# akshathmangudi/KAN-ViT

Measured on AMD Instinct MI355X. Metric: images/sec (train step) KAN-ViT 224x224, higher is better.
Workload: dtype f32

## Files before the change

include/kanvit.h:

```cpp
#ifndef KANVIT_H
#define KANVIT_H

#include <stddef.h>
#include <stdint.h>

#ifdef __cplusplus
extern "C" {
#endif

#if defined(__GNUC__) || defined(__clang__)
#pragma GCC visibility push(default)
#endif

#define KANVIT_ABI_VERSION 7

#define KANVIT_OK 0
#define KANVIT_EINVAL (-22)
#define KANVIT_ENOMEM (-12)
#define KANVIT_EDEVICE (-5)

#define KANVIT_FLAG_BF16_MFMA 1

#define KANVIT_FLAG_UNIFORM_KNOTS 2
#define KANVIT_FLAG_FUSED_LN 8
#define KANVIT_FLAG_SHARED_BPARAMS 4

#define KANVIT_FLAG_SINE_DFREQ 16

#define KANVIT_LINEAR 0
#define KANVIT_CHEBY 1
#define KANVIT_BSPLINE 2
#define KANVIT_RBF 3
#define KANVIT_SINE 4
#define KANVIT_FOURIER 5

typedef struct kanvit_layer_desc {
    int32_t family;
    int32_t groups;
    int32_t x_group_mod;
    int32_t I;
    int32_t O;
    int32_t G;
    int32_t spline_order;
    int32_t has_base;
    float rbf_inv_h;
    int32_t flags;
    int64_t M;
    int64_t ldx;
    int64_t ldu;
    int64_t ldy;
    int64_t bparam_stride;
    float ln_eps;
    int32_t base_act;
} kanvit_layer_desc;


#define KANVIT_BASE_SILU 0
#define KANVIT_BASE_GELU 1
#define KANVIT_BASE_GELU_TANH 2
#define KANVIT_BASE_RELU 3
#define KANVIT_BASE_TANH 4
#define KANVIT_BASE_IDENTITY 5

int kanvit_layer_ln_fusable(const kanvit_layer_desc* d);

size_t kanvit_layer_ln_bwd_workspace(const kanvit_layer_desc* d);
int kanvit_layer_ln_bwd(const kanvit_layer_desc* d, const float* x, const float* stats, const float* bparams, const float* du,
                        float* dx, float* dgamma, float* dbeta, void* workspace, size_t workspace_bytes, void* stream);

size_t kanvit_layer_fwd_workspace(const kanvit_layer_desc* d);
int kanvit_layer_fwd(const kanvit_layer_desc* d, const float* x, const float* u, const float* w,
                     const float* bparams, const float* bias, float* y, void* workspace, size_t workspace_bytes,
                     void* stream);

size_t kanvit_layer_bwd_input_workspace(const kanvit_layer_desc* d);
int kanvit_layer_bwd_input(const kanvit_layer_desc* d, const float* x, const float* u, const float* w,
                           const float* bparams, const float* dy, float* dx, float* du, float* dparam,
                           void* workspace, size_t workspace_bytes, void* stream);
int64_t kanvit_layer_dparam_tiles(const kanvit_layer_desc* d);
int kanvit_layer_sine_dfreq_ok(const kanvit_layer_desc* d);

size_t kanvit_layer_bwd_weight_workspace(const kanvit_layer_desc* d);
int kanvit_layer_bwd_weight(const kanvit_layer_desc* d, const float* x, const float* u, const float* bparams,
                            const float* dy, float* dw, void* workspace, size_t workspace_bytes, void* stream);

int kanvit_edge_l1_supported(const kanvit_layer_desc* d);
int64_t kanvit_edge_l1_row_bands(const kanvit_layer_desc* d);
size_t kanvit_edge_l1_fwd_workspace(const kanvit_layer_desc* d);
int kanvit_edge_l1_fwd(const kanvit_layer_desc* d, const float* x, const float* w, const float* bparams, float* A, void* workspace,
                       size_t workspace_bytes, void* stream);
size_t kanvit_edge_l1_bwd_workspace(const kanvit_layer_desc* d);
int kanvit_edge_l1_bwd(const kanvit_layer_desc* d, const float* x, const float* w, const float* bparams, const float* gA, float* dw,
                       float* dx, void* workspace, size_t workspace_bytes, void* stream);

#define KANVIT_BSPLINE_REFIT_TAU 1e-5
int kanvit_bspline_refit_supported(const kanvit_layer_desc* d);
size_t kanvit_bspline_refit_workspace(const kanvit_layer_desc* d);
int kanvit_bspline_refit_gram(const kanvit_layer_desc* d, const float* x, const float* old_knots, const float* new_knots, double* N,
                              double* C, void* workspace, size_t workspace_bytes, void* stream);
int kanvit_bspline_refit_solve(const kanvit_layer_desc* d, const double* N, const double* C, const float* w_old, float* w_new,
                               unsigned char* ok, void* stream);

int kanvit_bspline_regrid_supported(const kanvit_layer_desc* d, int old_G);
size_t kanvit_bspline_regrid_workspace(const kanvit_layer_desc* d, int old_G);
int kanvit_bspline_regrid_gram(const kanvit_layer_desc* d, int old_G, const float* x, const float* old_knots, const float* new_knots,
                               double* N, double* C, void* workspace, size_t workspace_bytes, void* stream);
int kanvit_bspline_regrid_solve(const kanvit_layer_desc* d, int old_G, const double* N, const double* C, const float* w_old,
                                float* w_new, unsigned char* ok, void* stream);

typedef struct kanvit_patch_desc {
    int32_t C, H, W;
    int32_t n_patches;
    int32_t prepend_rows;
    int32_t reserved;
} kanvit_patch_desc;
int kanvit_patch_embed_fwd(const kanvit_layer_desc* d, const kanvit_patch_desc* p, const float* images, const float* w,
                           const float* bparams, const float* bias, const float* cls, const float* pos, float* y,
                           void* stream);
int kanvit_patch_embed_fwd_ws(const kanvit_layer_desc* d, const kanvit_patch_desc* p, const float* images, const float* w,
                              const float* bparams, const float* bias, const float* cls, const float* pos, float* y,
                              void* workspace, size_t workspace_bytes, void* stream);
int kanvit_patch_embed_bwd_weight_ok(const kanvit_layer_desc* d, const kanvit_patch_desc* p);
size_t kanvit_patch_embed_bwd_weight_workspace(const kanvit_layer_desc* d, const kanvit_patch_desc* p);
int kanvit_patch_embed_bwd_weight(const kanvit_layer_desc* d, const kanvit_patch_desc* p, const float* images,
                                  const float* bparams, const float* dy, float* dw, void* workspace, size_t workspace_bytes,
                                  void* stream);

#define KANVIT_ATTN_MAX_N 256
#define KANVIT_ATTN_MAX_D 64
typedef struct kanvit_attn_desc {
    int32_t B, H, N, D;
    int32_t causal;
    float scale;
    int32_t flags;
    int32_t reserved;
    int64_t q_stride_b, q_stride_h, q_stride_n;
    int64_t k_stride_b, k_stride_h, k_stride_n;
    int64_t v_stride_b, v_stride_h, v_stride_n;
    int64_t o_stride_b, o_stride_h, o_stride_n;
} kanvit_attn_desc;

int kanvit_attn_fwd(const kanvit_attn_desc* d, const float* q, const float* k, const float* v,
                    float* o, float* lse, void* stream);
size_t kanvit_attn_bwd_workspace(const kanvit_attn_desc* d);
int kanvit_attn_bwd(const kanvit_attn_desc* d, const float* q, const float* k, const float* v,
                    const float* o, const float* lse, const float* d_o,
                    float* dq, float* dk, float* dv, void* workspace, size_t workspace_bytes, void* stream);

#define KANVIT_ATTN_X_MAX_D 128
typedef struct kanvit_attn_ext {
    int32_t Nk;
    int32_t reserved;
    const void* mask;
    int64_t mask_stride_b, mask_stride_h, mask_stride_q, mask_stride_k;
} kanvit_attn_ext;
int kanvit_attn_x_fwd(const kanvit_attn_desc* d, const kanvit_attn_ext* e, const float* q, const float* k, const float* v,
                      float* o, float* lse, void* stream);
size_t kanvit_attn_x_bwd_workspace(const kanvit_attn_desc* d, const kanvit_attn_ext* e);
int kanvit_attn_x_bwd(const kanvit_attn_desc* d, const kanvit_attn_ext* e, const float* q, const float* k, const float* v,
                      const float* o, const float* lse, const float* d_o, float* dq, float* dk, float* dv, void* workspace,
                      size_t workspace_bytes, void* stream);

int kanvit_attn_probs(const kanvit_attn_desc* d, const kanvit_attn_ext* e, const float* q, const float* k, float* p,
                      int64_t p_stride_b, int64_t p_stride_h, int64_t p_stride_q, int32_t rows, void* stream);

int kanvit_attn_q1_fwd(const kanvit_attn_desc* d, const kanvit_attn_ext* e, const float* q, const float* k, const float* v,
                       float* o, float* p, void* stream);
int kanvit_attn_q1_bwd(const kanvit_attn_desc* d, const kanvit_attn_ext* e, const float* q, const float* k, const float* v,
                       const float* o, const float* p, const float* d_o, float* dq, float* dk, float* dv, void* stream);

int kanvit_ff_small_supported(int D, int F);
int64_t kanvit_ff_small_max_rows(void);
int kanvit_ff_small_fwd(int64_t M, int D, int F, const float* x, const float* w1, const float* b1, const float* w2, const float* b2,
                        float* y, void* stream);
size_t kanvit_ff_small_bwd_workspace(int64_t M, int D, int F);
int kanvit_ff_small_bwd(int64_t M, int D, int F, const float* x, const float* w1, const float* b1, const float* w2, const float* dy,
                        float* dx, float* dw1, float* db1, float* dw2, float* db2, void* workspace, size_t workspace_bytes, void* stream);
int kanvit_lnff_small_fwd(int64_t M, int D, int F, float eps, const float* x, const float* delta, const float* gamma, const float* beta,
                          const float* w1, const float* b1, const float* w2, const float* b2, float* s, float* mean, float* rstd, float* y,
                          void* stream);
int kanvit_lnff_small_bwd(int64_t M, int D, int F, const float* s, const float* mean, const float* rstd, const float* gamma, const float* beta,
                          const float* w1, const float* b1, const float* w2, const float* dy, const float* ds_in, float* ds, float* dgamma,
                          float* dbeta, float* dw1, float* db1, float* dw2, float* db2, void* workspace, size_t workspace_bytes, void* stream);

int kanvit_addln_fwd(int64_t M, int D, float eps, const float* x, const float* delta, const float* gamma, const float* beta,
                     float* xsum, float* y, float* mean, float* rstd, void* stream);
size_t kanvit_addln_bwd_workspace(int64_t M, int D);
int kanvit_addln_bwd(int64_t M, int D, const float* xsum, const float* gamma, const float* mean, const float* rstd,
                     const float* dy, const float* dres, float* dx, float* dgamma, float* dbeta, void* workspace,
                     size_t workspace_bytes, void* stream);
int kanvit_addln_fwd_ex(int64_t M, int D, float eps, const float* x, const void* delta, int delta_bf16, const float* gamma, const float* beta,
                        float* xsum, void* y, int y_bf16, float* mean, float* rstd, void* stream);
int kanvit_addln_bwd_ex(int64_t M, int D, const float* xsum, const float* gamma, const float* mean, const float* rstd,
                        const void* dy, int dy_bf16, const float* dres, float* dx, void* dx_bf16, float* dgamma, float* dbeta, void* workspace,
                        size_t workspace_bytes, void* stream);

#define KANVIT_DEPTH_MAX_BRANCHES 64
int kanvit_depth_scales(int64_t B, int n_branch, const float* keep, uint64_t seed, uint64_t* counter, float* scales, void* stream);
int kanvit_addln_sd_fwd(int64_t M, int D, float eps, const float* x, const void* delta, int delta_bf16, const float* gamma, const float* beta,
                        float* xsum, void* y, int y_bf16, float* mean, float* rstd, const float* row_scale, int64_t rows_per_sample,
                        void* stream);
int kanvit_addln_sd_bwd(int64_t M, int D, const float* xsum, const float* gamma, const float* mean, const float* rstd,
                        const void* dy, int dy_bf16, const float* dres, float* dx, void* ddelta, int ddelta_bf16, float* dgamma, float* dbeta,
                        const float* row_scale, int64_t rows_per_sample, void* workspace, size_t workspace_bytes, void* stream);

size_t kanvit_relu_bwd_bias_workspace(int64_t M, int N);
int kanvit_relu_bwd_bias(int64_t M, int N, const float* dy, const float* y, float* dh, float* dbias, void* workspace,
                         size_t workspace_bytes, void* stream);
int kanvit_relu_bwd_bias_bf16(int64_t M, int N, const void* dy_bf16, const void* y_bf16, void* dh_bf16, float* dbias, void* workspace,
                              size_t workspace_bytes, void* stream);

int kanvit_split3_bf16(int64_t M, int K, const float* x, const float* bias, int relu, const void* mask_hi, int64_t mask_ld,
                       void* out, int pattern, void* stream);

int kanvit_augment_u8_supported(int64_t N, int H, int W, int C, int pad_y, int pad_x);
int kanvit_augment_u8(const uint8_t* images, const int64_t* labels, const int64_t* idx, const float* lut, float* out, int64_t* y_out,
                      int32_t* params_out, int64_t N, int64_t B, int H, int W, int C, int pad_y, int pad_x, int flip, uint64_t seed,
                      uint64_t epoch, void* stream);

int kanvit_mix_u8(const uint8_t* images, const int64_t* labels, const int64_t* idx, const float* lut, const int64_t* partner,
                  const float* weight, const int32_t* box, float* out, int64_t* y_out, int64_t* y2_out, float* w_out, int64_t N, int64_t B,
                  int H, int W, int C, int pad_y, int pad_x, int flip, uint64_t seed, uint64_t epoch, void* stream);

int kanvit_resample_u8_supported(int64_t N, int H, int W, int C, int OH, int OW);
int kanvit_resample_u8(const uint8_t* images, const int64_t* labels, const int64_t* idx, const float* lut, const int32_t* crop,
                       const int64_t* partner, const float* weight, const int32_t* box, float* out, int64_t* y_out, int64_t* y2_out,
                       float* w_out, int64_t N, int64_t B, int H, int W, int C, int OH, int OW, void* stream);

int kanvit_soft_ce(const float* logits, int64_t ld, const int64_t* y1, const int64_t* y2, const float* w, int64_t B, int C, float eps,
                   float* loss_rows, float* dlogits, float* loss, void* stream);

int kanvit_metrics_update(const void* logits, int logits_bf16, int64_t ld, const int64_t* labels, int64_t B, int C, int64_t n0, int64_t cap,
                          float* probs_t, int32_t* labels_out, int32_t* preds_out, int64_t* confusion, void* stream);
size_t kanvit_metrics_auc_pairs_workspace(int64_t n, int C);
int kanvit_metrics_auc_pairs(const float* probs_t, const int32_t* labels, int64_t n, int C, int64_t cap, int64_t* counts, void* workspace,
                             size_t workspace_bytes, void* stream);

#define KANVIT_OPTIM_MAX_TENSORS 80
#define KANVIT_OPTIM_CHUNK 4096
int kanvit_optim_max_tensors(void);
size_t kanvit_optim_sumsq_workspace(int n, const int64_t* numel);
int kanvit_optim_sumsq(int n, const void* const* grads, const int64_t* numel, void* workspace, size_t workspace_bytes, void* stream);
int kanvit_optim_begin(const void* partials, int64_t n_partials, double max_norm, int64_t* step, float* norm_coef, void* stream);
int kanvit_optim_adamw(int n, void* const* params, const void* const* grads, const int64_t* offsets, const int64_t* numel,
                       const int32_t* decay, float* exp_avg, float* exp_avg_sq, float* ema, int64_t state_numel, const float* table,
                       int64_t table_rows, const int64_t* step, const float* norm_coef, int has_wd, float b1, float ob1, float b2, float ob2,
                       float eps, float d, float od, void* stream);

#define KANVIT_DECLARE_FAMILY(name)                                                                           \
    int kanvit_##name##_fwd(const kanvit_layer_desc*, const float*, const float*, const float*, const float*, \
                            const float*, float*, void*, size_t, void*);                                      \
    int kanvit_##name##_bwd_input(const kanvit_layer_desc*, const float*, const float*, const float*,         \
                                  const float*, const float*, float*, float*, float*, void*, size_t, void*);  \
    int kanvit_##name##_bwd_weight(const kanvit_layer_desc*, const float*, const float*, const float*,        \
                                   const float*, float*, void*, size_t, void*);                               \
    int kanvit_##name##_qkv_fwd(const kanvit_layer_desc*, const float*, const float*, const float*,           \
                                const float*, const float*, float*, void*, size_t, void*);                    \
    int kanvit_##name##_qkv_bwd_input(const kanvit_layer_desc*, const float*, const float*, const float*,     \
                                      const float*, const float*, float*, float*, float*, void*, size_t,      \
                                      void*);                                                                 \
    int kanvit_##name##_qkv_bwd_weight(const kanvit_layer_desc*, const float*, const float*, const float*,    \
                                       const float*, float*, void*, size_t, void*);
KANVIT_DECLARE_FAMILY(linear)
KANVIT_DECLARE_FAMILY(cheby)
KANVIT_DECLARE_FAMILY(bspline)
KANVIT_DECLARE_FAMILY(rbf)
KANVIT_DECLARE_FAMILY(sine)
KANVIT_DECLARE_FAMILY(fourier)

int kanvit_abi_version(void);
const char* kanvit_last_error(void);
const char* kanvit_config(void);
int kanvit_config_reload(void);
int kanvit_device_count(void);

#if defined(__GNUC__) || defined(__clang__)
#pragma GCC visibility pop
#endif

#ifdef __cplusplus
}
#endif
#endif
```

kan-vit_amd/csrc/attention.hip:

```cpp
#include "attention_common.h"

#include <type_traits>

#include <stdlib.h>

namespace {

constexpr int ATHR = 256;
constexpr float LOG2E = 1.4426950408889634f;

typedef __bf16 bf16x8_t __attribute__((ext_vector_type(8)));
typedef __bf16 bf16x2_t __attribute__((ext_vector_type(2)));
typedef unsigned u32x4 __attribute__((ext_vector_type(4)));

__device__ __forceinline__ unsigned kv_pk(float lo, float hi) {
    bf16x2_t v = {(__bf16)lo, (__bf16)hi};
    return __builtin_bit_cast(unsigned, v);
}
__device__ __forceinline__ bf16x8_t kv_pack8(const float (&f)[8]) {
    const u32x4 u = {kv_pk(f[0], f[1]), kv_pk(f[2], f[3]), kv_pk(f[4], f[5]), kv_pk(f[6], f[7])};
    return __builtin_bit_cast(bf16x8_t, u);
}
__device__ __forceinline__ bf16x8_t kv_row8(const float* __restrict__ p) {
    float f[8];
// ... 1973 lines not shown
    if (int rc = kv_launch<KV>(kv_name, p.grid, threads, p.lds, a, st)) return rc;
    return kv_launch<DQ>(dq_name, p.grid_q, threads, p.lds_q, a, st);
}

int launch_bwd(const AttnArgs& a, const AttnBwdPlan& p, hipStream_t st) {
    return kv_pick<1, 2>(a.D <= 32 ? 1 : 2, [&](auto dt) {
        constexpr int DT = decltype(dt)::value;
        switch (p.form) {
            case ATTN_BWD_KV4_DQ3:
                return kv_pick<4, 8>(p.nkt, [&](auto n) {
                    return launch_pair<attn_bwd_kv4_kernel<2>, attn_bwd_dq3_kernel<2, decltype(n)::value>>("attn_bwd_kv4_kernel", "attn_bwd_dq3_kernel", 512, a, p, st);
                });
            case ATTN_BWD_KV3_DQ3:
                return kv_pick<2, 4, 8>(p.nkt, [&](auto n) {
                    constexpr int NKT = decltype(n)::value;
                    return launch_pair<attn_bwd_kv3_kernel<DT, NKT>, attn_bwd_dq3_kernel<DT, NKT>>("attn_bwd_kv3_kernel", "attn_bwd_dq3_kernel", 512, a, p, st);
                });
            case ATTN_BWD_KV2DS_DQ:
                return launch_pair<attn_bwd_kv2_kernel<DT, false, true>, attn_bwd_dq_kernel<DT>>("attn_bwd_kv2_kernel", "attn_bwd_dq_kernel", 512, a, p, st);
            case ATTN_BWD_KV2DS_DQ_BF16:
                return kv_pick<4, 8>(p.nkt, [&](auto n) {
                    return launch_pair<attn_bwd_kv2_kernel<DT, true, true>, attn_bwd_dq_bf16_kernel<DT, decltype(n)::value>>("attn_bwd_kv2_kernel", "attn_bwd_dq_bf16_kernel", 512, a, p, st);
                });
            case ATTN_BWD_KV2_Q2:
                return p.bf16 ? launch_pair<attn_bwd_kv2_kernel<DT, true, false>, attn_bwd_q2_kernel<DT, true>>("attn_bwd_kv2_kernel", "attn_bwd_q2_kernel", 512, a, p, st)
                              : launch_pair<attn_bwd_kv2_kernel<DT, false, false>, attn_bwd_q2_kernel<DT, false>>("attn_bwd_kv2_kernel", "attn_bwd_q2_kernel", 512, a, p, st);
            default:
                return p.bf16 ? launch_pair<attn_bwd_kv_kernel<DT, true>, attn_bwd_q_kernel<DT, true>>("attn_bwd_kv_kernel", "attn_bwd_q_kernel", ATHR, a, p, st)
                              : launch_pair<attn_bwd_kv_kernel<DT, false>, attn_bwd_q_kernel<DT, false>>("attn_bwd_kv_kernel", "attn_bwd_q_kernel", ATHR, a, p, st);
        }
    });
}

__device__ __forceinline__ void attn_small_store_row(float* __restrict__ rowp, const f32x16& acc, int hf, int D, float mul) {
#pragma unroll
    for (int r = 0; r < 16; ++r) {
        const int d = kv_acc_row(r, hf);
        if (d < D) rowp[d] = acc[r] * mul;
    }
}

__global__ __launch_bounds__(256) void attn_small_fwd_kernel(const AttnArgs a) {
    const int lane = threadIdx.x & 63, wave = threadIdx.x >> 6, l31 = lane & 31, hf = lane >> 5;
    const int bh = blockIdx.x * 4 + wave;
    if (bh >= a.B * a.H) return;
    const int bi = bh / a.H, hi = bh - bi * a.H;
    const int N = a.N, D = a.D, DHc = (D + 1) / 2;
    const bool row_ok = l31 < N;
    const float* qrow = a.q + bi * a.qsb + hi * a.qsh + (long long)(row_ok ? l31 : 0) * a.qsn;
    const float* krow = a.k + bi * a.ksb + hi * a.ksh + (long long)(row_ok ? l31 : 0) * a.ksn;
    const float* vb = a.v + bi * a.vsb + hi * a.vsh;
    float vt[16];
#pragma unroll
    for (int r = 0; r < 16; ++r) {
        const int key = kv_acc_row(r, hf);
        vt[r] = (key < N && l31 < D) ? vb[(long long)key * a.vsn + l31] : 0.0f;
    }
    f32x16 sacc;
#pragma unroll
    for (int r = 0; r < 16; ++r) sacc[r] = 0.0f;
    for (int s = 0; s < DHc; ++s) {
        const int d = hf * DHc + s;
        const bool ok = row_ok && d < D;
        sacc = __builtin_amdgcn_mfma_f32_32x32x2f32(ok ? krow[d] : 0.0f, ok ? qrow[d] : 0.0f, sacc, 0, 0, 0);
    }
    const float sc2 = a.scale * LOG2E;
    float mx = -INFINITY;
#pragma unroll
    for (int r = 0; r < 16; ++r) {
        const int key = kv_acc_row(r, hf);
        if (key >= N || (a.causal && key > l31)) sacc[r] = -INFINITY;
        mx = fmaxf(mx, sacc[r]);
    }
    mx = fmaxf(mx, __shfl_xor(mx, 32));
    float sum = 0.0f;
#pragma unroll
    for (int r = 0; r < 16; ++r) {
        const float p = exp2f((sacc[r] - mx) * sc2);
        sacc[r] = p;
        sum += p;
    }
    sum += __shfl_xor(sum, 32);
    f32x16 oacc;
#pragma unroll
    for (int r = 0; r < 16; ++r) oacc[r] = 0.0f;
#pragma unroll
    for (int r = 0; r < 16; ++r) oacc = __builtin_amdgcn_mfma_f32_32x32x2f32(vt[r], sacc[r], oacc, 0, 0, 0);
    if (row_ok) {
        attn_small_store_row(a.out + bi * a.osb + hi * a.osh + (long long)l31 * a.osn, oacc, hf, D, 1.0f / sum);
        if (hf == 0 && a.lse) a.lse[(long long)bh * N + l31] = mx * a.scale + logf(sum);
    }
}

__global__ __launch_bounds__(256) void attn_small_bwd_kernel(const AttnArgs a) {
    __shared__ float tiles[4][2][32 * 33];
    const int lane = threadIdx.x & 63, wave = threadIdx.x >> 6, l31 = lane & 31, hf = lane >> 5;
    const int bh = blockIdx.x * 4 + wave;
    if (bh >= a.B * a.H) return;
    const int bi = bh / a.H, hi = bh - bi * a.H;
    const int N = a.N, D = a.D, DHc = (D + 1) / 2;
    const bool row_ok = l31 < N;
    const long long r0 = row_ok ? l31 : 0;
    const float* qb = a.q + bi * a.qsb + hi * a.qsh;
    const float* kb = a.k + bi * a.ksb + hi * a.ksh;
    const float* vb = a.v + bi * a.vsb + hi * a.vsh;
    const float* ob = a.o + bi * a.osb + hi * a.osh;
    const float* dob = a.d_o + bi * a.osb + hi * a.osh;
    float kt[16], dot[16], qt[16];
#pragma unroll
    for (int r = 0; r < 16; ++r) {
        const int key = kv_acc_row(r, hf);
        kt[r] = (key < N && l31 < D) ? kb[(long long)key * a.ksn + l31] : 0.0f;
        const int qq = 2 * r + hf;
        const bool ok = qq < N && l31 < D;
        dot[r] = ok ? dob[(long long)qq * a.osn + l31] : 0.0f;
        qt[r] = ok ? qb[(long long)qq * a.qsn + l31] : 0.0f;
    }
    f32x16 sacc, pacc;
#pragma unroll
    for (int r = 0; r < 16; ++r) {
        sacc[r] = 0.0f;
        pacc[r] = 0.0f;
    }
    float dl = 0.0f;
    for (int s = 0; s < DHc; ++s) {
        const int d = hf * DHc + s;
        const bool ok = row_ok && d < D;
        const float kv = ok ? kb[r0 * a.ksn + d] : 0.0f, qv = ok ? qb[r0 * a.qsn + d] : 0.0f;
        const float vv = ok ? vb[r0 * a.vsn + d] : 0.0f, dv = ok ? dob[r0 * a.osn + d] : 0.0f;
        const float ov = ok ? ob[r0 * a.osn + d] : 0.0f;
        sacc = __builtin_amdgcn_mfma_f32_32x32x2f32(kv, qv, sacc, 0, 0, 0);
        pacc = __builtin_amdgcn_mfma_f32_32x32x2f32(vv, dv, pacc, 0, 0, 0);
        dl += dv * ov;
    }
    dl += __shfl_xor(dl, 32);
    const float sc2 = a.scale * LOG2E;
    const float lse2 = row_ok ? a.lse_in[(long long)bh * N + l31] * LOG2E : INFINITY;
    float* pt = tiles[wave][0];
    float* dst = tiles[wave][1];
#pragma unroll
    for (int r = 0; r < 16; ++r) {
        const int key = kv_acc_row(r, hf);
        float p = exp2f(sacc[r] * sc2 - lse2);
        if (key >= N || (a.causal && key > l31)) p = 0.0f;
        const float ds = p * a.scale * (pacc[r] - dl);
        sacc[r] = p;
        pacc[r] = ds;
        pt[key * 33 + l31] = p;
        dst[key * 33 + l31] = ds;
    }
    f32x16 dqacc, dkacc, dvacc;
#pragma unroll
    for (int r = 0; r < 16; ++r) {
        dqacc[r] = 0.0f;
        dkacc[r] = 0.0f;
        dvacc[r] = 0.0f;
    }
#pragma unroll
    for (int r = 0; r < 16; ++r) dqacc = __builtin_amdgcn_mfma_f32_32x32x2f32(kt[r], pacc[r], dqacc, 0, 0, 0);
    __builtin_amdgcn_wave_barrier();
#pragma unroll
    for (int r = 0; r < 16; ++r) {
        dvacc = __builtin_amdgcn_mfma_f32_32x32x2f32(dot[r], pt[l31 * 33 + 2 * r + hf], dvacc, 0, 0, 0);
        dkacc = __builtin_amdgcn_mfma_f32_32x32x2f32(qt[r], dst[l31 * 33 + 2 * r + hf], dkacc, 0, 0, 0);
    }
    if (row_ok) {
        attn_small_store_row(a.dq + bi * a.qsb + hi * a.qsh + (long long)l31 * a.qsn, dqacc, hf, D, 1.0f);
        attn_small_store_row(a.dk + bi * a.ksb + hi * a.ksh + (long long)l31 * a.ksn, dkacc, hf, D, 1.0f);
        attn_small_store_row(a.dv + bi * a.vsb + hi * a.vsh + (long long)l31 * a.vsn, dvacc, hf, D, 1.0f);
    }
}

struct AttnSwitches {
    bool v1, v2, v3, v4, no_ds, no_bf16;
    int grid;
};
AttnSwitches attn_switches() {
    const KvConfig& c = kv_config();
    return {c.attn_v1 != 0, c.attn_v2 != 0, c.attn_v3 != 0, c.attn_v4 != 0, c.attn_no_ds != 0, c.no_bf16 != 0, c.attn_grid};
}

unsigned grid_per_cu(int nbh, int per_cu, int grid_override) {
    const int g = grid_override > 0 ? grid_override : KV_N_CU * per_cu;
    return (unsigned)(nbh < g ? nbh : g);
}
unsigned grid_resident(int nbh, size_t lds, int grid_override) { return grid_per_cu(nbh, lds * 2 <= 160 * 1024 ? 2 : 1, grid_override); }

int nkt_bucket(int nkt) { return nkt <= 2 ? nkt : nkt <= 4 ? 4 : nkt <= 7 ? 7 : 8; }

}

AttnFwdPlan plan_attn_fwd(const kanvit_attn_desc* d, uintptr_t align) {
    const AttnSwitches sw = attn_switches();
    const int nbh = d->B * d->H, nkt = (d->N + 31) / 32, D = d->D <= 32 ? 32 : 64;
    const size_t NP = (size_t)nkt * 32;
    AttnFwdPlan p{};
    if (d->N <= 32 && d->D <= 32 && !sw.v1 && !sw.v2) {
        p.form = ATTN_FWD_SMALL;
        p.grid = (unsigned)((nbh + 3) / 4);
        return p;
    }
    p.bf16 = (d->flags & KANVIT_FLAG_BF16_MFMA) && d->D % 16 == 0 && !sw.no_bf16;
    const bool rows16 = desc_vec(d) && align % 16 == 0;
    const bool newest = rows16 && !sw.v1 && !sw.v2 && !sw.v3;
    const int t16 = kv_attn16_tiles(d);
    if (newest && !sw.v4 && !d->causal && t16 && (!p.bf16 || t16 == KV_ATTN16_TILES)) {
        p.form = p.bf16 ? ATTN_FWD_16_BF16 : ATTN_FWD_16;
        p.nkt = t16;
        p.lds = kv_attn16_fwd_lds(d->N);
        p.grid = grid_per_cu(nbh, 1, sw.grid);
    } else if (newest && !p.bf16 && d->D == 64 && nkt >= 3 && nkt <= 7 && kv_a4_lds(d->N, 64) <= 160 * 1024) {
        p.form = ATTN_FWD_FOURTH;
        p.nkt = nkt <= 4 ? 4 : 7;
        p.lds = kv_a4_lds(d->N, 64);
        p.grid = grid_per_cu(nbh, 1, sw.grid);
    } else if (rows16 && !p.bf16 && d->D == D && !sw.v1 && !sw.v2 && nkt <= 7) {
        p.form = ATTN_FWD_THIRD;
        p.nkt = nkt_bucket(nkt);
        p.lds = sizeof(float) * 2 * NP * kv_pad4(D);
        p.grid = grid_resident(nbh, p.lds, sw.grid);
    } else if (rows16 && d->D == D && !sw.v1 && nkt <= 7) {
        p.form = ATTN_FWD_SECOND;
        p.nkt = nkt_bucket(nkt);
        p.lds = p.bf16 ? sizeof(unsigned short) * (NP * (D + 8) + D * (NP + 8)) : sizeof(float) * 2 * NP * (D + 1);
        p.grid = (unsigned)nbh;
    } else {
        p.form = ATTN_FWD_FIRST;
        p.nkt = nkt_bucket(nkt);
        p.lds = sizeof(float) * (2 * NP * (D + 1) + (size_t)4 * 32 * (D + 1));
        p.grid = (unsigned)nbh;
    }
    return p;
}

AttnBwdPlan plan_attn_bwd(const kanvit_attn_desc* d, const AttnAlign& al) {
    const AttnSwitches sw = attn_switches();
    const int nbh = d->B * d->H, nkt = (d->N + 31) / 32, D = d->D <= 32 ? 32 : 64;
    const size_t NP = (size_t)nkt * 32;
    AttnBwdPlan p{};
    p.bf16 = (d->flags & KANVIT_FLAG_BF16_MFMA) && d->D % 16 == 0 && !sw.no_bf16;
    const bool want16 = !sw.v1 && !sw.v2 && !sw.v3 && !sw.v4 && !sw.no_ds && d->D == 64 && !d->causal && (d->N + 15) / 16 == KV_ATTN16_TILES;
    const bool ds = (d->D == 32 || d->D == 64) && !d->causal && !sw.no_ds && !sw.v1 && !(want16 && !p.bf16) && (!p.bf16 || d->N <= 256);
    p.ws_bytes = (sizeof(float) * (size_t)d->B * d->H * d->N + 15) / 16 * 16 + (ds ? (p.bf16 ? sizeof(unsigned short) : sizeof(float)) * (size_t)d->B * d->H * NP * NP : 0);
    p.grid = p.grid_q = (unsigned)nbh;
    if (d->N <= 32 && d->D <= 32 && !sw.v1 && !sw.v2) {
        p.form = ATTN_BWD_SMALL;
        p.bf16 = false;
        p.grid = (unsigned)((nbh + 3) / 4);
        return p;
    }
    const bool rows16 = desc_vec(d) && al.rows % 16 == 0;
    if (want16 && rows16 && kv_attn16_tiles(d) && al.o % 16 == 0 && al.lse % 4 == 0) {
        p.form = p.bf16 ? ATTN_BWD_16_BF16 : ATTN_BWD_16;
        p.nkt = KV_ATTN16_TILES;
        p.lds = kv_attn16_bwd_lds();
        p.grid = grid_per_cu(nbh, 1, sw.grid);
        return p;
    }
    const size_t lds3 = sizeof(float) * (2 * NP * kv_pad4(D) + 2 * NP), lds_dq3 = sizeof(float) * NP * kv_pad4(D);
    const bool third = ds && !p.bf16 && !sw.v2 && rows16 && al.o % 16 == 0 && lds3 <= 160 * 1024;
    p.delta = !third;
    const size_t row = sizeof(unsigned short) * NP * (D + 8), tr = sizeof(unsigned short) * D * (NP + 8), f32img = sizeof(float) * NP * (D + 1);
    const size_t lds_kv2 = (p.bf16 ? 2 * row + 2 * tr : 2 * f32img) + sizeof(float) * 2 * NP;
    if (!(rows16 && d->D == D && !sw.v1 && lds_kv2 <= 160 * 1024)) {
        p.form = ATTN_BWD_KV_Q;
        p.lds_q = sizeof(float) * (2 * NP * (D + 1) + (size_t)4 * 32 * (D + 1));
        p.lds = p.lds_q + sizeof(float) * 2 * NP;
    } else if (third && D == 64 && nkt >= 3 && nkt <= 7 && kv_b4_lds(d->N, 64) <= 160 * 1024 && !sw.v3) {
        p.form = ATTN_BWD_KV4_DQ3;
        p.nkt = nkt <= 4 ? 4 : 8;
        p.lds = kv_b4_lds(d->N, 64);
        p.grid = grid_per_cu(nbh, 1, sw.grid);
        p.lds_q = lds_dq3;
        p.grid_q = grid_resident(nbh, lds_dq3, sw.grid);
    } else if (third) {
        p.form = ATTN_BWD_KV3_DQ3;
        p.nkt = nkt <= 2 ? 2 : nkt <= 4 ? 4 : 8;
        p.lds = lds3;
        p.grid = grid_resident(nbh, lds3, sw.grid);
        p.lds_q = lds_dq3;
        p.grid_q = grid_resident(nbh, lds_dq3, sw.grid);
    } else if (ds) {
        p.form = p.bf16 ? ATTN_BWD_KV2DS_DQ_BF16 : ATTN_BWD_KV2DS_DQ;
        p.nkt = nkt <= 4 ? 4 : 8;
        p.lds = lds_kv2;
        p.lds_q = p.bf16 ? tr : f32img;
    } else {
        p.form = ATTN_BWD_KV2_Q2;
        p.lds = lds_kv2;
        p.lds_q = p.bf16 ? 2 * row + tr : 2 * f32img;
    }
    p.ds = p.form == ATTN_BWD_KV2DS_DQ_BF16 ? ATTN_DS_BF16 : p.form == ATTN_BWD_KV4_DQ3 || p.form == ATTN_BWD_KV3_DQ3 || p.form == ATTN_BWD_KV2DS_DQ ? ATTN_DS_F32 : ATTN_DS_NONE;
    return p;
}

extern "C" {

#ifdef KANVIT_CLOCK_PROBE
__attribute__((visibility("default"))) int kanvit_debug_clock(unsigned long long* out) {
    return hipMemcpyFromSymbol(out, HIP_SYMBOL(g_kv_clk), 10 * sizeof(unsigned long long)) == hipSuccess ? 0 : -5;
}
#endif

int kanvit_attn_fwd(const kanvit_attn_desc* d, const float* q, const float* k, const float* v, float* o, float* lse,
                    void* stream) {
    if (int rc = check_desc(d, "kanvit_attn_fwd")) return rc;
    if (!q || !k || !v || !o) return kv_fail(KANVIT_EINVAL, "kanvit_attn_fwd: null q/k/v/o");
    if (d->B == 0) return 0;
    AttnArgs a = make_args(d);
    a.q = q; a.k = k; a.v = v; a.out = o; a.lse = lse;
    a.vec = a.vec && (((uintptr_t)q | (uintptr_t)k | (uintptr_t)v) % 16 == 0);
    hipStream_t st = (hipStream_t)stream;
    const AttnFwdPlan p = plan_attn_fwd(d, (uintptr_t)q | (uintptr_t)k | (uintptr_t)v | (uintptr_t)o);
    switch (p.form) {
        case ATTN_FWD_SMALL:
            hipLaunchKernelGGL(attn_small_fwd_kernel, dim3(p.grid), dim3(256), 0, st, a);
            KV_LAUNCH_CHECK("attn_small_fwd_kernel");
            return 0;
        case ATTN_FWD_16:
        case ATTN_FWD_16_BF16:
            return kv_attn16_launch_fwd(a, p, st);
        default:
            return launch_fwd(a, p, st);
    }
}

size_t kanvit_attn_bwd_workspace(const kanvit_attn_desc* d) {
    if (!d || d->B < 0 || d->H < 1 || d->N < 1) return 0;
    return plan_attn_bwd(d, AttnAlign{}).ws_bytes;
}

int kanvit_attn_bwd(const kanvit_attn_desc* d, const float* q, const float* k, const float* v, const float* o,
                    const float* lse, const float* d_o, float* dq, float* dk, float* dv, void* workspace,
                    size_t workspace_bytes, void* stream) {
    if (int rc = check_desc(d, "kanvit_attn_bwd")) return rc;
    if (!q || !k || !v || !o || !lse || !d_o || !dq || !dk || !dv)
        return kv_fail(KANVIT_EINVAL, "kanvit_attn_bwd: null argument");
    if (d->B == 0) return 0;
    const uintptr_t in = (uintptr_t)q | (uintptr_t)k | (uintptr_t)v | (uintptr_t)d_o;
    const AttnBwdPlan p = plan_attn_bwd(d, AttnAlign{in | (uintptr_t)dq | (uintptr_t)dk | (uintptr_t)dv, (uintptr_t)o, (uintptr_t)lse});
    if (!workspace || workspace_bytes < p.ws_bytes)
        return kv_fail(KANVIT_ENOMEM, "kanvit_attn_bwd: workspace %zu bytes < required %zu", workspace_bytes, p.ws_bytes);
    AttnArgs a = make_args(d);
    a.q = q; a.k = k; a.v = v; a.o = o; a.lse_in = lse; a.d_o = d_o;
    a.dq = dq; a.dk = dk; a.dv = dv; a.delta = (float*)workspace; a.delta_in = a.delta;
    a.ds = p.ds != ATTN_DS_NONE ? (float*)((char*)workspace + (sizeof(float) * (size_t)d->B * d->H * d->N + 15) / 16 * 16) : nullptr;
    a.vec = a.vec && in % 16 == 0;
    a.third = !p.delta;
    hipStream_t st = (hipStream_t)stream;
    switch (p.form) {
        case ATTN_BWD_SMALL:
            hipLaunchKernelGGL(attn_small_bwd_kernel, dim3(p.grid), dim3(256), 0, st, a);
            KV_LAUNCH_CHECK("attn_small_bwd_kernel");
            return 0;
        case ATTN_BWD_16:
        case ATTN_BWD_16_BF16:
            return kv_attn16_launch_bwd(a, p, st);
        default:
            if (p.delta) {
                hipLaunchKernelGGL(attn_delta_kernel, dim3((unsigned)(((long long)d->B * d->H * d->N + 15) / 16)), dim3(256), 0, st, a);
                KV_LAUNCH_CHECK("attn_delta_kernel");
            }
            return launch_bwd(a, p, st);
    }
}

}
```

kan-vit_amd/csrc/attention16.hip:

```cpp
#include "attention_common.h"

#include <stdlib.h>

#include <type_traits>
#include <utility>

namespace {

template <int N, typename F, int... I>
__device__ __forceinline__ void a16_static_for_impl(F&& f, std::integer_sequence<int, I...>) { (f(std::integral_constant<int, I>{}), ...); }
template <int N, typename F>
__device__ __forceinline__ void a16_static_for(F&& f) { a16_static_for_impl<N>(f, std::make_integer_sequence<int, N>{}); }

typedef __attribute__((address_space(3))) void* a16_lds_ptr;
typedef const __attribute__((address_space(1))) void* a16_glb_ptr;

constexpr int A16_D = 64;
constexpr int A16_NW = 12;
constexpr int A16_THREADS = 64 * A16_NW;
constexpr int A16_MAXT = 13;
constexpr int A16_SCR = 1024 + 64 + 64 + 16;

__host__ __device__ constexpr int a16_rows(int N) { return (N + 3) & ~3; }
inline size_t a16_lds_bytes(int N) { return sizeof(float) * ((size_t)3 * a16_rows(N) * A16_D + A16_SCR); }
// ... 69 lines not shown
    const bool has_tile = wave < nt && wave < A16_NW;
    constexpr bool cut = nt > A16_NW;
    const bool cutw = cut && wave < 4;
    const int npieces = R >> 2;
    const int qrow = 16 * wave + m;
    const bool qok = has_tile && qrow < N;
    const int crow = 16 * A16_NW + m;
    const int kb0 = cutw ? (wave * nt) >> 2 : 0, kb1 = cutw ? ((wave + 1) * nt) >> 2 : 0;

    int koff[4], voff[4];
    auto make_koff = [&]() {
        int l = lane;
        asm volatile("" : "+v"(l));
        const int mm = l & 15, gg = l >> 4;
#pragma unroll
        for (int i = 0; i < 4; ++i) koff[i] = mm * D + 4 * ((4 * gg + i) ^ a16_f(mm));
    };
    auto make_voff = [&]() {
        int l = lane;
        asm volatile("" : "+v"(l));
        const int mm = l & 15, gg = l >> 4;
#pragma unroll
        for (int r = 0; r < 4; ++r) voff[r] = (4 * gg + r) * D + 4 * (mm ^ a16_f(4 * gg + r));
    };
    constexpr int jl = nt - 1;

    float qf[16];
    auto load_q = [&](int bh) {
        const int bi = bh / a.H, hi = bh - bi * a.H;
        int l = lane;
        asm volatile("" : "+v"(l));
        const int qr = 16 * wave + (l & 15);
        const float* qp = a.q + bi * a.qsb + hi * a.qsh + (qr < N ? qr : 0) * (int)a.qsn + 16 * (l >> 4);
#pragma unroll
        for (int i = 0; i < 4; ++i) {
            const f32x4 u = *reinterpret_cast<const f32x4*>(qp + 4 * i);
#pragma unroll
            for (int e = 0; e < 4; ++e) qf[4 * i + e] = u[e];
        }
    };
    auto fill = [&](int item, const float* base, long long sn) {
        a16_fill(smem + (item % 3) * IMG, base, (int)sn, 0, npieces, N, wave, A16_NW, lane);
    };
    auto fill_q12 = [&](int bh) {
        if (cut && wave >= 4 && wave < 8) {
            const int bi = bh / a.H, hi = bh - bi * a.H;
            a16_fill(q12_s, a.q + bi * a.qsb + hi * a.qsh, (int)a.qsn, 16 * A16_NW, 4, N, wave - 4, 4, lane);
        }
    };

    f32x4 oacc[4];
    float o_inv = 0.0f, o_lse = 0.0f;
    int o_bh = -1;
    auto store_o = [&]() {
        if (o_bh >= 0) {
            if (qok) {
                const int bi = o_bh / a.H, hi = o_bh - bi * a.H;
                int l = lane;
                asm volatile("" : "+v"(l));
                float* op = a.out + bi * a.osb + hi * a.osh + (16 * wave + (l & 15)) * (int)a.osn + 16 * (l >> 4);
#pragma unroll
                for (int r = 0; r < 4; ++r) {
                    const f32x4 v = {oacc[0][r] * o_inv, oacc[1][r] * o_inv, oacc[2][r] * o_inv, oacc[3][r] * o_inv};
                    *reinterpret_cast<f32x4*>(op + 4 * r) = v;
                }
                if (l < 16 && a.lse) a.lse[(long long)o_bh * N + 16 * wave + l] = o_lse;
            }
            o_bh = -1;
        }
    };

    for (int e = tid * 4; e < 3 * IMG + A16_SCR; e += A16_THREADS * 4) *reinterpret_cast<f32x4*>(smem + e) = f32x4{0.0f, 0.0f, 0.0f, 0.0f};
    __syncthreads();
    int item = 0;
    unsigned cut_done = 0;
    int bh = blockIdx.x;
    if (bh < nbh) {
        const int bi = bh / a.H, hi = bh - bi * a.H;
        fill(0, a.k + bi * a.ksb + hi * a.ksh, a.ksn);
        fill_q12(bh);
        if (has_tile) load_q(bh);
    }
    for (; bh < nbh; bh += gridDim.x) {
        const int bi = bh / a.H, hi = bh - bi * a.H;
        asm volatile("s_waitcnt vmcnt(0)" ::: "memory");
#pragma unroll
        for (int e = 0; e < 16; ++e) asm volatile("" : "+v"(qf[e]));
        __builtin_amdgcn_s_barrier();
        fill(item + 1, a.v + bi * a.vsb + hi * a.vsh, a.vsn);
        const float* K_s = smem + (item % 3) * IMG;
        make_koff();
        f32x4 sacc[NKT];
        a16_bf8 pbs[BF ? (NKT + 1) / 2 : 1];
        float inv = 0.0f, lse_v = 0.0f;
        if (has_tile) {
#pragma unroll
            for (int j = 0; j < NKT; ++j) sacc[j] = f32x4{0.0f, 0.0f, 0.0f, 0.0f};
            if constexpr (BF) {
                const a16_bf8 qb0 = a16_pack8(qf[0], qf[1], qf[2], qf[3], qf[4], qf[5], qf[6], qf[7]);
                const a16_bf8 qb1 = a16_pack8(qf[8], qf[9], qf[10], qf[11], qf[12], qf[13], qf[14], qf[15]);
#pragma unroll
                for (int j = 0; j < NKT; ++j) {
                    f32x4 ka[4];
#pragma unroll
                    for (int i = 0; i < 4; ++i) ka[i] = *reinterpret_cast<const f32x4*>(K_s + koff[i] + j * 16 * D);
                    sacc[j] = a16_mfma_bf(a16_pack8(ka[0][0], ka[0][1], ka[0][2], ka[0][3], ka[1][0], ka[1][1], ka[1][2], ka[1][3]), qb0, sacc[j]);
                    sacc[j] = a16_mfma_bf(a16_pack8(ka[2][0], ka[2][1], ka[2][2], ka[2][3], ka[3][0], ka[3][1], ka[3][2], ka[3][3]), qb1, sacc[j]);
                    if (j & 1) __builtin_amdgcn_sched_barrier(0);
                }
            } else {
                constexpr int NG = ((NKT + 1) / 2) * 4;
                f32x4 fa[3], fb[3];
                auto rd = [&](auto tc, f32x4& xa, f32x4& xb) {
                    constexpr int t = decltype(tc)::value, j = 2 * (t >> 2), i = t & 3;
                    xa = *reinterpret_cast<const f32x4*>(K_s + koff[i] + j * 16 * D);
                    if constexpr (j + 1 < NKT) xb = *reinterpret_cast<const f32x4*>(K_s + koff[i] + (j + 1) * 16 * D);
                };
                rd(std::integral_constant<int, 0>{}, fa[0], fb[0]);
                rd(std::integral_constant<int, 1>{}, fa[1], fb[1]);
                a16_static_for<NG>([&](auto tc) {
                    constexpr int t = decltype(tc)::value, j = 2 * (t >> 2), i = t & 3;
                    if constexpr (t + 2 < NG) rd(std::integral_constant<int, t + 2>{}, fa[(t + 2) % 3], fb[(t + 2) % 3]);
                    __builtin_amdgcn_sched_barrier(0);
#pragma unroll
                    for (int e = 0; e < 4; ++e) {
                        sacc[j] = a16_mfma(fa[t % 3][e], qf[4 * i + e], sacc[j]);
                        if constexpr (j + 1 < NKT) sacc[j + 1] = a16_mfma(fb[t % 3][e], qf[4 * i + e], sacc[j + 1]);
                    }
                    __builtin_amdgcn_sched_barrier(0);
                });
            }
            const int lim = CAUSAL ? (qrow + 1 < N ? qrow + 1 : N) : N;
            float mx = -INFINITY;
#pragma unroll
            for (int j = 0; j < NKT; ++j) {
                if (CAUSAL || j == jl) {
#pragma unroll
                    for (int r = 0; r < 4; ++r) sacc[j][r] = (16 * j + 4 * g + r >= lim) ? -INFINITY : sacc[j][r];
                }
#pragma unroll
                for (int r = 0; r < 4; ++r) mx = fmaxf(mx, sacc[j][r]);
            }
            mx = a16_gmax(mx);
            const float mxs = (mx == -INFINITY) ? 0.0f : mx * sc2;
            float sum = 0.0f;
#pragma unroll
            for (int j = 0; j < NKT; ++j) {
#pragma unroll
                for (int r = 0; r < 4; ++r) {
                    const float p = __builtin_amdgcn_exp2f(sacc[j][r] * sc2 - mxs);
                    sacc[j][r] = p;
                    sum += p;
                }
            }
            sum = a16_gsum(sum);
            inv = 1.0f / sum;
            lse_v = mx * a.scale + logf(sum);
            if constexpr (BF) {
#pragma unroll
                for (int t = 0; t < (NKT + 1) / 2; ++t) {
                    constexpr int JL = NKT - 1;
                    const bool pair = 2 * t + 1 < NKT;
                    const int j1 = pair ? 2 * t + 1 : JL;
                    pbs[t] = a16_pack8(sacc[2 * t][0], sacc[2 * t][1], sacc[2 * t][2], sacc[2 * t][3], pair ? sacc[j1][0] : 0.0f, pair ? sacc[j1][1] : 0.0f,
                                       pair ? sacc[j1][2] : 0.0f, pair ? sacc[j1][3] : 0.0f);
                }
            }
        }
        store_o();
        f32x4 cacc[4];
        if (cutw) {
            float cq[16];
#pragma unroll
            for (int i = 0; i < 4; ++i) {
                const f32x4 u = *reinterpret_cast<const f32x4*>(q12_s + koff[i]);
#pragma unroll
                for (int e = 0; e < 4; ++e) cq[4 * i + e] = u[e];
            }
            const int clim = CAUSAL ? (crow + 1 < N ? crow + 1 : N) : N;
#pragma unroll
            for (int jj = 0; jj < 4; ++jj) cacc[jj] = f32x4{0.0f, 0.0f, 0.0f, 0.0f};
            const float* Kq = K_s + kb0 * 16 * D;
            auto cut_s = [&](auto j0c, auto twoc) {
                constexpr int j0 = decltype(j0c)::value;
                constexpr bool two = decltype(twoc)::value;
                f32x4 ka[4], kb[4];
#pragma unroll
                for (int i = 0; i < 4; ++i) {
                    ka[i] = *reinterpret_cast<const f32x4*>(Kq + koff[i] + j0 * 16 * D);
                    if constexpr (two) kb[i] = *reinterpret_cast<const f32x4*>(Kq + koff[i] + (j0 + 1) * 16 * D);
                }
#pragma unroll
                for (int i = 0; i < 4; ++i)
#pragma unroll
                    for (int e = 0; e < 4; ++e) {
                        cacc[j0] = a16_mfma(ka[i][e], cq[4 * i + e], cacc[j0]);
                        if constexpr (two) cacc[j0 + 1] = a16_mfma(kb[i][e], cq[4 * i + e], cacc[j0 + 1]);
                    }
            };
            if constexpr (BF) {
                const a16_bf8 qb0 = a16_pack8(cq[0], cq[1], cq[2], cq[3], cq[4], cq[5], cq[6], cq[7]);
                const a16_bf8 qb1 = a16_pack8(cq[8], cq[9], cq[10], cq[11], cq[12], cq[13], cq[14], cq[15]);
#pragma unroll
                for (int jj = 0; jj < 4; ++jj) {
                    if (jj < 3 || kb1 - kb0 == 4) {
                        f32x4 ka[4];
#pragma unroll
                        for (int i = 0; i < 4; ++i) ka[i] = *reinterpret_cast<const f32x4*>(Kq + koff[i] + jj * 16 * D);
                        cacc[jj] = a16_mfma_bf(a16_pack8(ka[0][0], ka[0][1], ka[0][2], ka[0][3], ka[1][0], ka[1][1], ka[1][2], ka[1][3]), qb0, cacc[jj]);
                        cacc[jj] = a16_mfma_bf(a16_pack8(ka[2][0], ka[2][1], ka[2][2], ka[2][3], ka[3][0], ka[3][1], ka[3][2], ka[3][3]), qb1, cacc[jj]);
                    }
                }
            } else {
                cut_s(std::integral_constant<int, 0>{}, std::true_type{});
                if (kb1 - kb0 == 4) cut_s(std::integral_constant<int, 2>{}, std::true_type{});
                else cut_s(std::integral_constant<int, 2>{}, std::false_type{});
            }
            float mx = -INFINITY;
#pragma unroll
            for (int jj = 0; jj < 4; ++jj) {
                const int j = kb0 + jj;
                if (CAUSAL || jj >= 2) {
#pragma unroll
                    for (int r = 0; r < 4; ++r) cacc[jj][r] = (j >= kb1 || 16 * j + 4 * g + r >= clim) ? -INFINITY : cacc[jj][r];
                }
#pragma unroll
                for (int r = 0; r < 4; ++r) mx = fmaxf(mx, cacc[jj][r]);
            }
            mx = a16_gmax(mx);
            if (g == 0) mx4_s[wave * 16 + m] = mx;
        }
        ++item;
        asm volatile("s_waitcnt vmcnt(0)" ::: "memory");
        __builtin_amdgcn_s_barrier();
        const int bhn = bh + gridDim.x;
        if (bhn < nbh) {
            const int bn = bhn / a.H, hn = bhn - bn * a.H;
            fill(item + 1, a.k + bn * a.ksb + hn * a.ksh, a.ksn);
            fill_q12(bhn);
            if (has_tile) load_q(bhn);
        }
        const float* V_s = smem + (item % 3) * IMG;
        make_voff();
        float* const part_s = smem + ((item + 2) % 3) * IMG;
        if (cutw) {
            const float mx = fmaxf(fmaxf(mx4_s[m], mx4_s[16 + m]), fmaxf(mx4_s[32 + m], mx4_s[48 + m]));
            const float mxs = (mx == -INFINITY) ? 0.0f : mx * sc2;
            float sum = 0.0f;
            f32x4 pacc[4];
#pragma unroll
            for (int dt = 0; dt < 4; ++dt) pacc[dt] = f32x4{0.0f, 0.0f, 0.0f, 0.0f};
#pragma unroll
            for (int jj = 0; jj < 4; ++jj)
#pragma unroll
                for (int r = 0; r < 4; ++r) {
                    const float p = __builtin_amdgcn_exp2f(cacc[jj][r] * sc2 - mxs);
                    cacc[jj][r] = p;
                    sum += p;
                }
            const float* Vq = V_s + kb0 * 16 * D;
            auto cut_pv = [&](auto ngc) {
                constexpr int NGC = decltype(ngc)::value;
                f32x4 fv[3];
                fv[0] = *reinterpret_cast<const f32x4*>(Vq + voff[0]);
                fv[1] = *reinterpret_cast<const f32x4*>(Vq + voff[1]);
                a16_static_for<NGC>([&](auto tc) {
                    constexpr int t = decltype(tc)::value, jj = t >> 2, r = t & 3;
                    if constexpr (t + 2 < NGC) fv[(t + 2) % 3] = *reinterpret_cast<const f32x4*>(Vq + voff[(t + 2) & 3] + ((t + 2) >> 2) * 16 * D);
                    __builtin_amdgcn_sched_barrier(0);
#pragma unroll
                    for (int dt = 0; dt < 4; ++dt) pacc[dt] = a16_mfma(fv[t % 3][dt], cacc[jj][r], pacc[dt]);
                    __builtin_amdgcn_sched_barrier(0);
                });
            };
            if constexpr (BF) {
#pragma unroll
                for (int t = 0; t < 2; ++t) {
                    f32x4 v[8];
#pragma unroll
                    for (int r = 0; r < 4; ++r) {
                        v[r] = *reinterpret_cast<const f32x4*>(Vq + voff[r] + (2 * t) * 16 * D);
                        v[4 + r] = *reinterpret_cast<const f32x4*>(Vq + voff[r] + (2 * t + 1) * 16 * D);
                    }
                    const a16_bf8 pb = a16_pack8(cacc[2 * t][0], cacc[2 * t][1], cacc[2 * t][2], cacc[2 * t][3], cacc[2 * t + 1][0], cacc[2 * t + 1][1],
                                                 cacc[2 * t + 1][2], cacc[2 * t + 1][3]);
#pragma unroll
                    for (int dt = 0; dt < 4; ++dt)
                        pacc[dt] = a16_mfma_bf(a16_pack8(v[0][dt], v[1][dt], v[2][dt], v[3][dt], v[4][dt], v[5][dt], v[6][dt], v[7][dt]), pb, pacc[dt]);
                }
            } else {
                if (kb1 - kb0 == 4) cut_pv(std::integral_constant<int, 16>{});
                else cut_pv(std::integral_constant<int, 12>{});
            }
            sum = a16_gsum(sum);
            if (g == 0) sum4_s[wave * 16 + m] = sum;
#pragma unroll
            for (int r = 0; r < 4; ++r) {
                const f32x4 v = {pacc[0][r], pacc[1][r], pacc[2][r], pacc[3][r]};
                *reinterpret_cast<f32x4*>(part_s + ((wave * 4 + r) * 64 + lane) * 4) = v;
            }
            asm volatile("s_waitcnt lgkmcnt(0)" ::: "memory");
            a16_signal(cnt_s, lane);
        }
        if (has_tile) {
#pragma unroll
            for (int dt = 0; dt < 4; ++dt) oacc[dt] = f32x4{0.0f, 0.0f, 0.0f, 0.0f};
            if constexpr (BF) {
#pragma unroll
                for (int t = 0; t < (NKT + 1) / 2; ++t) {
                    constexpr int JL = NKT - 1;
                    const int j1 = (2 * t + 1 < NKT) ? 2 * t + 1 : JL;
                    f32x4 v[8];
#pragma unroll
                    for (int r = 0; r < 4; ++r) {
                        v[r] = *reinterpret_cast<const f32x4*>(V_s + voff[r] + (2 * t) * 16 * D);
                        v[4 + r] = *reinterpret_cast<const f32x4*>(V_s + voff[r] + j1 * 16 * D);
                    }
#pragma unroll
                    for (int dt = 0; dt < 4; ++dt)
                        oacc[dt] = a16_mfma_bf(a16_pack8(v[0][dt], v[1][dt], v[2][dt], v[3][dt], v[4][dt], v[5][dt], v[6][dt], v[7][dt]), pbs[t], oacc[dt]);
                    __builtin_amdgcn_sched_barrier(0);
                }
            } else {
                constexpr int NGV = 4 * NKT;
                f32x4 fv[3];
                auto rdv = [&](auto tc, f32x4& x) {
                    constexpr int t = decltype(tc)::value, j = t >> 2, r = t & 3;
                    x = *reinterpret_cast<const f32x4*>(V_s + voff[r] + j * 16 * D);
                };
                rdv(std::integral_constant<int, 0>{}, fv[0]);
                rdv(std::integral_constant<int, 1>{}, fv[1]);
                a16_static_for<NGV>([&](auto tc) {
                    constexpr int t = decltype(tc)::value, j = t >> 2, r = t & 3;
                    if constexpr (t + 2 < NGV) rdv(std::integral_constant<int, t + 2>{}, fv[(t + 2) % 3]);
                    __builtin_amdgcn_sched_barrier(0);
#pragma unroll
                    for (int dt = 0; dt < 4; ++dt) oacc[dt] = a16_mfma(fv[t % 3][dt], sacc[j][r], oacc[dt]);
                    __builtin_amdgcn_sched_barrier(0);
                });
            }
            o_bh = bh;
            o_inv = inv;
            o_lse = lse_v;
        }
        if (cutw) {
            ++cut_done;
            a16_wait(cnt_s, 4u * cut_done);
            f32x4 t = *reinterpret_cast<const f32x4*>(part_s + ((0 * 4 + wave) * 64 + lane) * 4);
#pragma unroll
            for (int q = 1; q < 4; ++q) t += *reinterpret_cast<const f32x4*>(part_s + ((q * 4 + wave) * 64 + lane) * 4);
            const float mx = fmaxf(fmaxf(mx4_s[m], mx4_s[16 + m]), fmaxf(mx4_s[32 + m], mx4_s[48 + m]));
            const float sum = ((sum4_s[m] + sum4_s[16 + m]) + sum4_s[32 + m]) + sum4_s[48 + m];
            const float cinv = 1.0f / sum;
            int l = lane;
            asm volatile("" : "+v"(l));
            const int cl = 16 * A16_NW + (l & 15);
            if (cl < N) {
                *reinterpret_cast<f32x4*>(a.out + bi * a.osb + hi * a.osh + cl * (int)a.osn + 16 * (l >> 4) + 4 * wave) = t * cinv;
                if (wave == 0 && l < 16 && a.lse) a.lse[(long long)bh * N + cl] = mx * a.scale + logf(sum);
            }
        }
        ++item;
    }
    store_o();
}

template <int NKT, bool BF>
int launch_fwd16(const AttnArgs& a, const AttnFwdPlan& p, hipStream_t st) {
    KV_ALLOW_LDS(160 * 1024, (attn16_fwd_kernel<NKT, false, BF>));
    hipLaunchKernelGGL((attn16_fwd_kernel<NKT, false, BF>), dim3(p.grid), dim3(A16_THREADS), p.lds, st, a);
    KV_LAUNCH_CHECK("attn16_fwd_kernel");
    return 0;
}

#ifndef B16_ABLATE
#define B16_ABLATE 0
#endif
#ifdef KANVIT_CLOCK_PROBE
#ifndef B16_CLK_WAVE
#define B16_CLK_WAVE 0
#endif
__device__ unsigned long long g_b16_clk[16];
#define B16_CLK_BEGIN() unsigned long long b16_t0 = 0, b16_r0 = 0, b16_tp = 0, b16_ph[14] = {0, 0, 0, 0, 0, 0, 0, 0, 0, 0, 0, 0, 0, 0}; \
    const bool b16_stamp = (blockIdx.x == gridDim.x / 2) && wave == B16_CLK_WAVE && lane == 0;                      \
    if (b16_stamp) { b16_t0 = b16_tp = __builtin_amdgcn_s_memtime(); b16_r0 = __builtin_amdgcn_s_memrealtime(); }
#define B16_CLK_PHASE(i) if (b16_stamp) { __builtin_amdgcn_sched_barrier(0); const unsigned long long b16_now = __builtin_amdgcn_s_memtime(); b16_ph[i] += b16_now - b16_tp; b16_tp = b16_now; __builtin_amdgcn_sched_barrier(0); }
#define B16_CLK_END() if (b16_stamp) { g_b16_clk[0] = __builtin_amdgcn_s_memtime() - b16_t0; g_b16_clk[1] = __builtin_amdgcn_s_memrealtime() - b16_r0; \
    for (int b16_i = 0; b16_i < 14; ++b16_i) g_b16_clk[2 + b16_i] = b16_ph[b16_i]; }
#else
#define B16_CLK_BEGIN()
#define B16_CLK_PHASE(i)
#define B16_CLK_END()
#endif
constexpr int B16_NW = 8;
constexpr int B16_THREADS = 64 * B16_NW;
constexpr int B16_NT = 13;
constexpr int B16_SL = 3 * 1024 + 64 + 16;
constexpr int B16_NSL = 6;
constexpr int B16_AHEAD = 4;
constexpr int B16_DST = 16 * 17;
constexpr int B16_DSS = B16_NT * B16_DST;
constexpr int B16_NDS = 4;
constexpr int B16_LAG = 2;
constexpr int B16_PART = 2 * 1024;
constexpr int B16_NPT = 2;
constexpr int B16_NCNT = 32;
enum { BC_READY = 0, BC_DELTA = 6, BC_DONE = 12, BC_DSW = 18, BC_DSR = 22, BC_PW = 26, BC_PR = 28 };
constexpr int b16_lds_floats() { return B16_NDS * B16_DSS + B16_NPT * B16_PART + B16_NSL * B16_SL + B16_NCNT; }

__device__ __forceinline__ void b16_wait(const unsigned* c, unsigned target) {
    if constexpr (!(B16_ABLATE & 32)) a16_wait(c, target);
}
__device__ __forceinline__ void b16_signal(unsigned* c, int lane, unsigned n = 1u) { a16_signal(c, lane, n); }

template <int NTL, bool BF>
__device__ __forceinline__ void attn16_bwd_body(const AttnArgs& a, float* __restrict__ smem, const int lane, const int wave) {
    constexpr int D = A16_D;
    constexpr bool UNITS = (NTL == 1);
    const int N = a.N, nbh = a.B * a.H;
    float* const dsr_s = smem;
    float* const part_s = dsr_s + B16_NDS * B16_DSS;
    float* const slices = part_s + B16_NPT * B16_PART;
    unsigned* const cnt = reinterpret_cast<unsigned*>(slices + B16_NSL * B16_SL);
    const float sc2 = a.scale * KV_LOG2E;
    const int nh = (nbh - (int)blockIdx.x + (int)gridDim.x - 1) / (int)gridDim.x;
    const int T = B16_NT * nh;
    const int kt0 = UNITS ? 10 + (wave - 5) : 2 * wave;
    const int u = wave - 5;

    auto head_of = [&](int k) { return (int)blockIdx.x + k * (int)gridDim.x; };
    auto slot6 = [&](int X) { return X % B16_NSL; };

    auto issue_slice = [&](int X) {
        if constexpr (!UNITS) {
            int l = lane;
            asm volatile("" : "+v"(l));
            const int k = X / B16_NT, sq = X - k * B16_NT;
            const int bh = head_of(k), bi = bh / a.H, hi = bh - bi * a.H;
            float* sl = slices + slot6(X) * B16_SL;
            const int lq = l >> 4;
#pragma unroll
            for (int c = 0; c < 3; ++c) {
                const int p = wave + 5 * c;
                if (p < 12) {
                    const int which = p >> 2, pp = p & 3;
                    int row = 16 * sq + 4 * pp + lq;
                    const int ls = (l & 15) ^ a16_f(4 * pp + lq);
                    row = row < N ? row : N - 1;
                    const float* src = which == 0 ? a.q + bi * a.qsb + hi * a.qsh + row * (int)a.qsn
                                                  : (which == 1 ? a.d_o : a.o) + bi * a.osb + hi * a.osh + row * (int)a.osn;
                    __builtin_amdgcn_global_load_lds((a16_glb_ptr)(src + 4 * ls), (a16_lds_ptr)(sl + which * 1024 + pp * 256), 16, 0, 0);
                } else if (p == 12) {
                    int row = 16 * sq + l;
                    row = row < N ? row : N - 1;
                    __builtin_amdgcn_global_load_lds((a16_glb_ptr)(a.lse_in + (long long)bh * N + row), (a16_lds_ptr)(sl + 3072), 4, 0, 0);
                }
            }
        }
    };
    auto form_delta = [&](int X) {
        int l = lane;
        asm volatile("" : "+v"(l));
        float* sl = slices + slot6(X) * B16_SL;
        const int row = l >> 2, part = l & 3;
        float dl = 0.0f;
#pragma unroll
        for (int j = 0; j < 4; ++j) {
            const int jr = (j + row) & 3;
            const f32x4 d4 = *reinterpret_cast<const f32x4*>(sl + 1024 + row * D + 16 * part + 4 * jr);
            const f32x4 o4 = *reinterpret_cast<const f32x4*>(sl + 2048 + row * D + 16 * part + 4 * jr);
            dl += d4[0] * o4[0] + d4[1] * o4[1] + d4[2] * o4[2] + d4[3] * o4[3];
        }
        dl += __shfl_xor(dl, 1);
        dl += __shfl_xor(dl, 2);
        if (part == 0) sl[3072 + 64 + row] = dl;
    };

    float kf[NTL][16], vf[NTL][16];
    a16_bf8 kfb[NTL][2], vfb[NTL][2];
    auto load_kv = [&](int k) {
        int l = lane;
        asm volatile("" : "+v"(l));
        const int bh = head_of(k), bi = bh / a.H, hi = bh - bi * a.H;
#pragma unroll
        for (int t = 0; t < NTL; ++t) {
            int key = 16 * (kt0 + t) + (l & 15);
            key = key < N ? key : N - 1;
            const float* kp = a.k + bi * a.ksb + hi * a.ksh + key * (int)a.ksn + 16 * (l >> 4);
            const float* vp = a.v + bi * a.vsb + hi * a.vsh + key * (int)a.vsn + 16 * (l >> 4);
#pragma unroll
            for (int i = 0; i < 4; ++i) {
                const f32x4 k4 = *reinterpret_cast<const f32x4*>(kp + 4 * i);
                const f32x4 v4 = *reinterpret_cast<const f32x4*>(vp + 4 * i);
#pragma unroll
                for (int e = 0; e < 4; ++e) {
                    kf[t][4 * i + e] = k4[e];
                    vf[t][4 * i + e] = v4[e];
                }
            }
            if constexpr (BF) {
#pragma unroll
                for (int c = 0; c < 2; ++c) {
                    kfb[t][c] = a16_pack8(kf[t][8 * c], kf[t][8 * c + 1], kf[t][8 * c + 2], kf[t][8 * c + 3], kf[t][8 * c + 4], kf[t][8 * c + 5], kf[t][8 * c + 6], kf[t][8 * c + 7]);
                    vfb[t][c] = a16_pack8(vf[t][8 * c], vf[t][8 * c + 1], vf[t][8 * c + 2], vf[t][8 * c + 3], vf[t][8 * c + 4], vf[t][8 * c + 5], vf[t][8 * c + 6], vf[t][8 * c + 7]);
                }
            }
        }
    };
    auto unit_tile = [&](int it) -> int { return it < 4 ? u + 3 * it : (u == 1 ? B16_NT - 1 : B16_NT); };
    float ku[UNITS ? 5 : 1][16];
    a16_s4 kub[UNITS ? 5 : 1][4];
    auto load_ku = [&](int k) {
        if constexpr (UNITS) {
            int l = lane;
            asm volatile("" : "+v"(l));
            const int bh = head_of(k), bi = bh / a.H, hi = bh - bi * a.H;
            const float* kb = a.k + bi * a.ksb + hi * a.ksh + 4 * (l & 15);
#pragma unroll
            for (int it = 0; it < 5; ++it) {
                const int kt = unit_tile(it);
                if (kt < B16_NT) {
#pragma unroll
                    for (int ks = 0; ks < 4; ++ks) {
                        int key = 16 * kt + 4 * (l >> 4) + ks;
                        key = key < N ? key : N - 1;
                        const f32x4 k4 = *reinterpret_cast<const f32x4*>(kb + key * (int)a.ksn);
#pragma unroll
                        for (int dt = 0; dt < 4; ++dt) ku[it][4 * ks + dt] = k4[dt];
                    }
                    if constexpr (BF) {
#pragma unroll
                        for (int dt = 0; dt < 4; ++dt) kub[it][dt] = a16_pack4(ku[it][dt], ku[it][4 + dt], ku[it][8 + dt], ku[it][12 + dt]);
                    }
                }
            }
        }
    };

    f32x4 dk[NTL][4], dv[NTL][4];
    auto zero_acc = [&]() {
#pragma unroll
        for (int t = 0; t < NTL; ++t)
#pragma unroll
            for (int dt = 0; dt < 4; ++dt) {
                dk[t][dt] = f32x4{0.0f, 0.0f, 0.0f, 0.0f};
                dv[t][dt] = f32x4{0.0f, 0.0f, 0.0f, 0.0f};
            }
    };
    auto store_dkv = [&](int k) {
        int l = lane;
        asm volatile("" : "+v"(l));
        const int bh = head_of(k), bi = bh / a.H, hi = bh - bi * a.H;
#pragma unroll
        for (int t = 0; t < NTL; ++t) {
            const int key = 16 * (kt0 + t) + (l & 15);
            if (key < N) {
                float* kp = a.dk + bi * a.ksb + hi * a.ksh + key * (int)a.ksn + 16 * (l >> 4);
                float* vp = a.dv + bi * a.vsb + hi * a.vsh + key * (int)a.vsn + 16 * (l >> 4);
#pragma unroll
                for (int r = 0; r < 4; ++r) {
                    *reinterpret_cast<f32x4*>(kp + 4 * r) = f32x4{dk[t][0][r], dk[t][1][r], dk[t][2][r], dk[t][3][r]};
                    *reinterpret_cast<f32x4*>(vp + 4 * r) = f32x4{dv[t][0][r], dv[t][1][r], dv[t][2][r], dv[t][3][r]};
                }
            }
        }
    };

    if constexpr (!UNITS) {
        for (int X = 0; X < B16_AHEAD && X < T; ++X) issue_slice(X);
    } else {
        load_ku(0);
    }
    load_kv(0);
    zero_acc();
    asm volatile("s_waitcnt vmcnt(0)" ::: "memory");
    __syncthreads();
    if (wave == 0) form_delta(0);
    if (threadIdx.x == 0) {
        for (int X = 0; X < B16_AHEAD; ++X) cnt[BC_READY + X] = 5u;
        cnt[BC_DELTA + 0] = 1u;
    }
    __syncthreads();

    auto peek = [&](const unsigned* c) -> unsigned { return *(const volatile a16_lds_u32*)c; };

    f32x4 dqp[UNITS ? 4 : 1];
    auto reduce_dq = [&](int Yp) {
        if constexpr (UNITS) {
            const int pslot = Yp & 1, ky = Yp / B16_NT, sy = Yp - ky * B16_NT;
            const float* pp = part_s + pslot * B16_PART;
            b16_wait(cnt + BC_PW + pslot, 2u * (unsigned)((Yp >> 1) + 1));
            int l = lane;
            asm volatile("" : "+v"(l));
            const int bh = head_of(ky), bi = bh / a.H, hi = bh - bi * a.H;
            const int q = 16 * sy + (l & 15);
            float* qp = a.dq + bi * a.qsb + hi * a.qsh + q * (int)a.qsn + 16 * (l >> 4);
            f32x4 p6[4], p7[4];
#pragma unroll
            for (int r = 0; r < 4; ++r) {
                p6[r] = *reinterpret_cast<const f32x4*>(pp + (r * 64 + l) * 4);
                p7[r] = *reinterpret_cast<const f32x4*>(pp + 1024 + (r * 64 + l) * 4);
            }
            b16_signal(cnt + BC_PR + pslot, lane);
#pragma unroll
            for (int r = 0; r < 4; ++r) {
                f32x4 t = dqp[r];
                t += p6[r];
                t += p7[r];
                if (q < N) *reinterpret_cast<f32x4*>(qp + 4 * r) = t;
            }
        }
    };

    int k = 0, s = 0;
    B16_CLK_BEGIN()
    for (int G = 0; G < T + B16_LAG; ++G) {
        B16_CLK_PHASE(7)
        if constexpr (UNITS) {
            asm volatile("s_waitcnt vmcnt(0)" ::: "memory");
            B16_CLK_PHASE(11)
            if (u == 0 && G >= B16_LAG + 1) reduce_dq(G - B16_LAG - 1);
            if (G >= B16_LAG) {
                const int Y = G - B16_LAG, dslot = Y % B16_NDS, pslot = Y & 1;
                const int ky = Y / B16_NT, sy = Y - ky * B16_NT;
                b16_wait(cnt + BC_DSW + dslot, (unsigned)B16_NT * (unsigned)(Y / B16_NDS + 1));
                B16_CLK_PHASE(8)
                int l = lane;
                asm volatile("" : "+v"(l));
                const int mm = l & 15, gg = l >> 4;
                f32x4 dq[4];
#pragma unroll
                for (int dt = 0; dt < 4; ++dt) dq[dt] = f32x4{0.0f, 0.0f, 0.0f, 0.0f};
                const float* dsb = dsr_s + dslot * B16_DSS + mm * 17 + 4 * gg;
                float b[5][4];
#pragma unroll
                for (int it = 0; it < 5; ++it)
                    if (unit_tile(it) < B16_NT) {
#pragma unroll
                        for (int ks = 0; ks < 4; ++ks) b[it][ks] = dsb[unit_tile(it) * B16_DST + ks];
                    }
#pragma unroll
                for (int it = 0; it < 5; ++it)
                    if (unit_tile(it) < B16_NT) {
                        if constexpr (BF) {
                            const a16_s4 bb = a16_pack4(b[it][0], b[it][1], b[it][2], b[it][3]);
#pragma unroll
                            for (int dt = 0; dt < 4; ++dt) dq[dt] = a16_mfma_bf4(kub[it][dt], bb, dq[dt]);
                        } else {
#pragma unroll
                            for (int ks = 0; ks < 4; ++ks)
#pragma unroll
                                for (int dt = 0; dt < 4; ++dt) {
                                    if constexpr (!(B16_ABLATE & 4)) dq[dt] = a16_mfma(ku[it][4 * ks + dt], b[it][ks], dq[dt]);
                                    else dq[dt][0] += ku[it][4 * ks + dt] * b[it][ks];
                                }
                        }
                    }
                B16_CLK_PHASE(9)
                b16_signal(cnt + BC_DSR + dslot, lane);
                if (sy == B16_NT - 1 && ky + 1 < nh) load_ku(ky + 1);
                B16_CLK_PHASE(13)
                if (u != 0) {
                    float* pp = part_s + pslot * B16_PART;
                    b16_wait(cnt + BC_PR + pslot, (unsigned)(Y >> 1));
                    B16_CLK_PHASE(6)
#pragma unroll
                    for (int r = 0; r < 4; ++r)
                        *reinterpret_cast<f32x4*>(pp + (u - 1) * 1024 + (r * 64 + l) * 4) = f32x4{dq[0][r], dq[1][r], dq[2][r], dq[3][r]};
                    b16_signal(cnt + BC_PW + pslot, lane);
                } else {
#pragma unroll
                    for (int r = 0; r < 4; ++r) dqp[r] = f32x4{dq[0][r], dq[1][r], dq[2][r], dq[3][r]};
                }
            }
        }
        if (G >= T) continue;
        if constexpr (!UNITS) {
            if (G + 1 < T && wave == (G + 1) % 5) {
                b16_wait(cnt + BC_READY + slot6(G + 1), 5u * (unsigned)((G + 1) / B16_NSL + 1));
                form_delta(G + 1);
                b16_signal(cnt + BC_DELTA + slot6(G + 1), lane);
            }
        }
        B16_CLK_PHASE(0)
        {
            const int slot = slot6(G), dslot = G % B16_NDS;
            const float* sl = slices + slot * B16_SL;
            b16_wait(cnt + BC_READY + slot, 5u * (unsigned)(G / B16_NSL + 1));
            B16_CLK_PHASE(1)
            int l = lane;
            asm volatile("" : "+v"(l));
            const int mm = l & 15, gg = l >> 4;
            int ko[4], vo[4];
#pragma unroll
            for (int i = 0; i < 4; ++i) ko[i] = mm * D + 4 * ((4 * gg + i) ^ a16_f(mm));
#pragma unroll
            for (int r = 0; r < 4; ++r) vo[r] = (4 * gg + r) * D + 4 * (mm ^ a16_f(4 * gg + r));
            f32x4 fq[4], fd[4], fo[4], fq2[4];
#pragma unroll
            for (int i = 0; i < 4; ++i) {
                fq[i] = *reinterpret_cast<const f32x4*>(sl + ko[i]);
                fd[i] = *reinterpret_cast<const f32x4*>(sl + 1024 + ko[i]);
            }
            const f32x4 ls4 = *reinterpret_cast<const f32x4*>(sl + 3072 + 4 * gg);
#pragma unroll
            for (int r = 0; r < 4; ++r) {
                fo[r] = *reinterpret_cast<const f32x4*>(sl + 1024 + vo[r]);
                fq2[r] = *reinterpret_cast<const f32x4*>(sl + vo[r]);
            }
            const unsigned dsr_seen = peek(cnt + BC_DSR + dslot);
            f32x4 sS[NTL], sP[NTL];
#pragma unroll
            for (int t = 0; t < NTL; ++t) {
                sS[t] = f32x4{0.0f, 0.0f, 0.0f, 0.0f};
                sP[t] = f32x4{0.0f, 0.0f, 0.0f, 0.0f};
            }
            if constexpr (BF) {
#pragma unroll
                for (int c = 0; c < 2; ++c) {
                    const a16_bf8 aq = a16_pack8(fq[2 * c][0], fq[2 * c][1], fq[2 * c][2], fq[2 * c][3], fq[2 * c + 1][0], fq[2 * c + 1][1], fq[2 * c + 1][2], fq[2 * c + 1][3]);
                    const a16_bf8 ad = a16_pack8(fd[2 * c][0], fd[2 * c][1], fd[2 * c][2], fd[2 * c][3], fd[2 * c + 1][0], fd[2 * c + 1][1], fd[2 * c + 1][2], fd[2 * c + 1][3]);
#pragma unroll
                    for (int t = 0; t < NTL; ++t) {
                        sS[t] = a16_mfma_bf(aq, kfb[t][c], sS[t]);
                        sP[t] = a16_mfma_bf(ad, vfb[t][c], sP[t]);
                    }
                }
            } else
#pragma unroll
            for (int i = 0; i < 4; ++i)
#pragma unroll
                for (int e = 0; e < 4; ++e)
#pragma unroll
                    for (int t = 0; t < NTL; ++t) {
                        if constexpr (!(B16_ABLATE & 1)) {
                            sS[t] = a16_mfma(fq[i][e], kf[t][4 * i + e], sS[t]);
                            sP[t] = a16_mfma(fd[i][e], vf[t][4 * i + e], sP[t]);
                        } else if (i == 0 && e == 0) {
                            sS[t][0] += fq[0][0] * kf[t][0] + fq[1][1] + fq[2][2] + fq[3][3];
                            sP[t][0] += fd[0][0] * vf[t][0] + fd[1][1] + fd[2][2] + fd[3][3];
                        }
                    }
            B16_CLK_PHASE(2)
            const bool last_s = (s == B16_NT - 1);
            if (last_s && k + 1 < nh) load_kv(k + 1);
            b16_wait(cnt + BC_DELTA + slot, (unsigned)(G / B16_NSL + 1));
            const f32x4 dl4 = *reinterpret_cast<const f32x4*>(sl + 3072 + 64 + 4 * gg);
            float pr[NTL][4], ds[NTL][4];
#pragma unroll
            for (int t = 0; t < NTL; ++t)
#pragma unroll
                for (int r = 0; r < 4; ++r) {
                    float p = __builtin_amdgcn_exp2f(sS[t][r] * sc2 - ls4[r] * KV_LOG2E);
                    const bool dead = (last_s && 16 * s + 4 * gg + r >= N) || (kt0 + t == B16_NT - 1 && 16 * (kt0 + t) + mm >= N);
                    p = dead ? 0.0f : p;
                    pr[t][r] = p;
                    ds[t][r] = p * (sP[t][r] - dl4[r]) * a.scale;
                }
            B16_CLK_PHASE(3)
            if constexpr (BF) {
                a16_s4 pb[NTL], db[NTL];
#pragma unroll
                for (int t = 0; t < NTL; ++t) {
                    pb[t] = a16_pack4(pr[t][0], pr[t][1], pr[t][2], pr[t][3]);
                    db[t] = a16_pack4(ds[t][0], ds[t][1], ds[t][2], ds[t][3]);
                }
#pragma unroll
                for (int dt = 0; dt < 4; ++dt) {
                    const a16_s4 ao = a16_pack4(fo[0][dt], fo[1][dt], fo[2][dt], fo[3][dt]);
                    const a16_s4 aq2 = a16_pack4(fq2[0][dt], fq2[1][dt], fq2[2][dt], fq2[3][dt]);
#pragma unroll
                    for (int t = 0; t < NTL; ++t) {
                        dv[t][dt] = a16_mfma_bf4(ao, pb[t], dv[t][dt]);
                        dk[t][dt] = a16_mfma_bf4(aq2, db[t], dk[t][dt]);
                    }
                }
            } else
#pragma unroll
            for (int r = 0; r < 4; ++r)
#pragma unroll
                for (int dt = 0; dt < 4; ++dt)
#pragma unroll
                    for (int t = 0; t < NTL; ++t) {
                        if constexpr (!(B16_ABLATE & 2)) {
                            dv[t][dt] = a16_mfma(fo[r][dt], pr[t][r], dv[t][dt]);
                            dk[t][dt] = a16_mfma(fq2[r][dt], ds[t][r], dk[t][dt]);
                        } else {
                            dv[t][dt][0] += fo[r][dt] * pr[t][r];
                            dk[t][dt][0] += fq2[r][dt] * ds[t][r];
                        }
                    }
            B16_CLK_PHASE(4)
            b16_signal(cnt + BC_DONE + slot, lane);
            if (G >= B16_NDS && dsr_seen < 3u * (unsigned)(G / B16_NDS)) b16_wait(cnt + BC_DSR + dslot, 3u * (unsigned)(G / B16_NDS));
            B16_CLK_PHASE(10)
            float* dsw = dsr_s + dslot * B16_DSS + (4 * gg) * 17 + mm;
#pragma unroll
            for (int t = 0; t < NTL; ++t)
#pragma unroll
                for (int r = 0; r < 4; ++r) dsw[(kt0 + t) * B16_DST + r * 17] = ds[t][r];
            b16_signal(cnt + BC_DSW + dslot, lane, (unsigned)NTL);
            if (last_s) {
                store_dkv(k);
                zero_acc();
            }
        }
        B16_CLK_PHASE(5)
        if constexpr (!UNITS) {
            const int XL = G + B16_AHEAD - 1, XI = G + B16_AHEAD;
            if (XL >= B16_AHEAD && XL < T) {
                asm volatile("s_waitcnt vmcnt(0)" ::: "memory");
                b16_signal(cnt + BC_READY + slot6(XL), lane);
            }
            B16_CLK_PHASE(11)
            if (XI < T && !(B16_ABLATE & 16)) {
                if (XI >= B16_NSL) b16_wait(cnt + BC_DONE + slot6(XI), (unsigned)B16_NW * (unsigned)(XI / B16_NSL));
                B16_CLK_PHASE(12)
                issue_slice(XI);
            }
        }
        B16_CLK_PHASE(6)
        if (++s == B16_NT) { s = 0; ++k; }
    }
    if constexpr (UNITS) {
        if (u == 0) reduce_dq(T - 1);
    }
    B16_CLK_END()
}

template <bool BF>
__global__ __launch_bounds__(B16_THREADS) void attn16_bwd_kernel(const AttnArgs a) {
    extern __shared__ __attribute__((aligned(16))) float smem[];
    const int tid = threadIdx.x, lane = tid & 63, wave = __builtin_amdgcn_readfirstlane(tid >> 6);
    for (int e = tid * 4; e < b16_lds_floats(); e += B16_THREADS * 4) *reinterpret_cast<f32x4*>(smem + e) = f32x4{0.0f, 0.0f, 0.0f, 0.0f};
    __syncthreads();
    if (wave < 5) attn16_bwd_body<2, BF>(a, smem, lane, wave);
    else attn16_bwd_body<1, BF>(a, smem, lane, wave);
}

static_assert(B16_NT == KV_ATTN16_TILES && A16_MAXT == KV_ATTN16_TILES && sizeof(float) * b16_lds_floats() <= 160 * 1024, "the backward's tiles and LDS");

}

int kv_attn16_tiles(const kanvit_attn_desc* d) {
    if (d->D != A16_D || d->N <= 64 || a16_lds_bytes(d->N) > 160 * 1024 || (d->N + 15) / 16 > A16_MAXT) return 0;
    for (long long sn : {d->q_stride_n, d->k_stride_n, d->v_stride_n, d->o_stride_n})
        if (sn * (long long)(d->N + 1) >= (1LL << 31)) return 0;
    return (d->N + 15) / 16;
}
size_t kv_attn16_fwd_lds(int N) { return a16_lds_bytes(N); }
size_t kv_attn16_bwd_lds() { return sizeof(float) * (size_t)b16_lds_floats(); }

int kv_attn16_launch_fwd(const AttnArgs& a, const AttnFwdPlan& p, hipStream_t st) {
    if (p.bf16) return launch_fwd16<A16_MAXT, true>(a, p, st);
    switch (p.nkt) {
        case 5: return launch_fwd16<5, false>(a, p, st);
        case 6: return launch_fwd16<6, false>(a, p, st);
        case 7: return launch_fwd16<7, false>(a, p, st);
        case 8: return launch_fwd16<8, false>(a, p, st);
        case 9: return launch_fwd16<9, false>(a, p, st);
        case 10: return launch_fwd16<10, false>(a, p, st);
        case 11: return launch_fwd16<11, false>(a, p, st);
        case 12: return launch_fwd16<12, false>(a, p, st);
        default: return launch_fwd16<13, false>(a, p, st);
    }
}

#ifdef KANVIT_CLOCK_PROBE
extern "C" __attribute__((visibility("default"))) int kanvit_debug_clock16(unsigned long long* out) {
    return hipMemcpyFromSymbol(out, HIP_SYMBOL(g_b16_clk), 16 * sizeof(unsigned long long)) == hipSuccess ? 0 : -5;
}
#endif

template <bool BF>
static int launch_bwd16(const AttnArgs& a, const AttnBwdPlan& p, hipStream_t st) {
    KV_ALLOW_LDS(160 * 1024, attn16_bwd_kernel<BF>);
    hipLaunchKernelGGL(attn16_bwd_kernel<BF>, dim3(p.grid), dim3(B16_THREADS), p.lds, st, a);
    KV_LAUNCH_CHECK("attn16_bwd_kernel");
    return 0;
}
int kv_attn16_launch_bwd(const AttnArgs& a, const AttnBwdPlan& p, hipStream_t st) { return p.bf16 ? launch_bwd16<true>(a, p, st) : launch_bwd16<false>(a, p, st); }
```

kan-vit_amd/csrc/attention_common.h:

```cpp
#pragma once
#include "kanvit_common.h"

struct AttnArgs {
    const float* q;
    const float* k;
    const float* v;
    const float* o;
    const float* lse_in;
    const float* d_o;
    const float* delta_in;
    float* out;
    float* lse;
    float* dq;
    float* dk;
    float* dv;
    float* delta;
    float* ds;
    long long qsb, qsh, qsn, ksb, ksh, ksn, vsb, vsh, vsn, osb, osh, osn;
    int B, H, N, D, causal, nkt, vec;
    int third;
    float scale;
};

constexpr int KV_N_CU = 256;
constexpr float KV_LOG2E = 1.4426950408889634f;

enum AttnFwdForm { ATTN_FWD_SMALL, ATTN_FWD_16, ATTN_FWD_16_BF16, ATTN_FWD_FOURTH, ATTN_FWD_THIRD, ATTN_FWD_SECOND, ATTN_FWD_FIRST };
enum AttnBwdForm { ATTN_BWD_SMALL, ATTN_BWD_16, ATTN_BWD_16_BF16, ATTN_BWD_KV4_DQ3, ATTN_BWD_KV3_DQ3, ATTN_BWD_KV2DS_DQ, ATTN_BWD_KV2DS_DQ_BF16,
                   ATTN_BWD_KV2_Q2, ATTN_BWD_KV_Q };
enum AttnDs { ATTN_DS_NONE, ATTN_DS_F32, ATTN_DS_BF16 };

struct AttnFwdPlan {
    AttnFwdForm form;
    bool bf16;
    int nkt;
    unsigned grid;
    size_t lds;
};

struct AttnBwdPlan {
    AttnBwdForm form;
    bool bf16;
    int nkt;
    unsigned grid, grid_q;
    size_t lds, lds_q;
    bool delta;
    AttnDs ds;
    size_t ws_bytes;
};

struct AttnAlign {
    uintptr_t rows;
    uintptr_t o;
    uintptr_t lse;
};

AttnFwdPlan plan_attn_fwd(const kanvit_attn_desc* d, uintptr_t align);
AttnBwdPlan plan_attn_bwd(const kanvit_attn_desc* d, const AttnAlign& al);

constexpr int KV_ATTN16_TILES = 13;
int kv_attn16_tiles(const kanvit_attn_desc* d);
size_t kv_attn16_fwd_lds(int N);
size_t kv_attn16_bwd_lds();
int kv_attn16_launch_fwd(const AttnArgs& a, const AttnFwdPlan& p, hipStream_t st);
int kv_attn16_launch_bwd(const AttnArgs& a, const AttnBwdPlan& p, hipStream_t st);
```

kan-vit_amd/kanvit/_lib.py:

```python
import ctypes as C
import os

import torch

HERE = os.path.dirname(os.path.abspath(__file__))
LIB_PATH = os.environ.get("KANVIT_LIB") or os.path.join(HERE, "libkanvit.so")

LINEAR, CHEBY, BSPLINE, RBF, SINE, FOURIER = range(6)
FLAG_BF16_MFMA = 1
FLAG_UNIFORM_KNOTS = 2
FLAG_SHARED_BPARAMS = 4
FLAG_FUSED_LN = 8
FLAG_SINE_DFREQ = 16
FAMILY_NAMES = ["linear", "cheby", "bspline", "rbf", "sine", "fourier"]
BASE_SILU, BASE_GELU, BASE_GELU_TANH, BASE_RELU, BASE_TANH, BASE_IDENTITY = range(6)
BASE_NAMES = ["silu", "gelu", "gelu-tanh", "relu", "tanh", "identity"]


class KanvitError(RuntimeError):
    pass


class LayerDesc(C.Structure):
    _fields_ = [("family", C.c_int32), ("groups", C.c_int32), ("x_group_mod", C.c_int32), ("I", C.c_int32),
                ("O", C.c_int32), ("G", C.c_int32), ("spline_order", C.c_int32), ("has_base", C.c_int32),
                ("rbf_inv_h", C.c_float), ("flags", C.c_int32), ("M", C.c_int64), ("ldx", C.c_int64),
                ("ldu", C.c_int64), ("ldy", C.c_int64), ("bparam_stride", C.c_int64), ("ln_eps", C.c_float), ("base_act", C.c_int32)]


class AttnDesc(C.Structure):
    _fields_ = [("B", C.c_int32), ("H", C.c_int32), ("N", C.c_int32), ("D", C.c_int32), ("causal", C.c_int32),
                ("scale", C.c_float), ("flags", C.c_int32), ("reserved", C.c_int32),
                ("q_stride_b", C.c_int64), ("q_stride_h", C.c_int64), ("q_stride_n", C.c_int64),
                ("k_stride_b", C.c_int64), ("k_stride_h", C.c_int64), ("k_stride_n", C.c_int64),
                ("v_stride_b", C.c_int64), ("v_stride_h", C.c_int64), ("v_stride_n", C.c_int64),
                ("o_stride_b", C.c_int64), ("o_stride_h", C.c_int64), ("o_stride_n", C.c_int64)]


class AttnExt(C.Structure):
    _fields_ = [("Nk", C.c_int32), ("reserved", C.c_int32), ("mask", C.c_void_p),
                ("mask_stride_b", C.c_int64), ("mask_stride_h", C.c_int64), ("mask_stride_q", C.c_int64), ("mask_stride_k", C.c_int64)]


class PatchDesc(C.Structure):
    _fields_ = [("C", C.c_int32), ("H", C.c_int32), ("W", C.c_int32), ("n_patches", C.c_int32), ("prepend_rows", C.c_int32),
                ("reserved", C.c_int32)]


_P = C.c_void_p
_LAYER_FWD = [C.POINTER(LayerDesc), _P, _P, _P, _P, _P, _P, _P, C.c_size_t, _P]
_LAYER_BWD_IN = [C.POINTER(LayerDesc), _P, _P, _P, _P, _P, _P, _P, _P, _P, C.c_size_t, _P]
_LAYER_BWD_W = [C.POINTER(LayerDesc), _P, _P, _P, _P, _P, _P, C.c_size_t, _P]

SYMBOLS = {
    "kanvit_abi_version": (C.c_int, []),
    "kanvit_last_error": (C.c_char_p, []),
    "kanvit_device_count": (C.c_int, []),
    "kanvit_config": (C.c_char_p, []),
    "kanvit_config_reload": (C.c_int, []),
    "kanvit_ff_small_supported": (C.c_int, [C.c_int, C.c_int]),
    "kanvit_ff_small_max_rows": (C.c_int64, []),
    "kanvit_ff_small_fwd": (C.c_int, [C.c_int64, C.c_int, C.c_int] + [C.c_void_p] * 7),
    "kanvit_ff_small_bwd_workspace": (C.c_size_t, [C.c_int64, C.c_int, C.c_int]),
    "kanvit_ff_small_bwd": (C.c_int, [C.c_int64, C.c_int, C.c_int] + [C.c_void_p] * 11 + [C.c_size_t, C.c_void_p]),
    "kanvit_lnff_small_fwd": (C.c_int, [C.c_int64, C.c_int, C.c_int, C.c_float] + [C.c_void_p] * 13),
    "kanvit_lnff_small_bwd": (C.c_int, [C.c_int64, C.c_int, C.c_int] + [C.c_void_p] * 18 + [C.c_size_t, C.c_void_p]),
    "kanvit_layer_ln_fusable": (C.c_int, [C.POINTER(LayerDesc)]),
    "kanvit_layer_ln_bwd_workspace": (C.c_size_t, [C.POINTER(LayerDesc)]),
    "kanvit_layer_ln_bwd": (C.c_int, [C.POINTER(LayerDesc)] + [C.c_void_p] * 8 + [C.c_size_t, C.c_void_p]),
    "kanvit_layer_fwd_workspace": (C.c_size_t, [C.POINTER(LayerDesc)]),
    "kanvit_layer_bwd_input_workspace": (C.c_size_t, [C.POINTER(LayerDesc)]),
    "kanvit_layer_fwd": (C.c_int, _LAYER_FWD),
    "kanvit_layer_bwd_input": (C.c_int, _LAYER_BWD_IN),
    "kanvit_layer_dparam_tiles": (C.c_int64, [C.POINTER(LayerDesc)]),
    "kanvit_layer_sine_dfreq_ok": (C.c_int, [C.POINTER(LayerDesc)]),
    "kanvit_layer_bwd_weight_workspace": (C.c_size_t, [C.POINTER(LayerDesc)]),
    "kanvit_layer_bwd_weight": (C.c_int, _LAYER_BWD_W),
    "kanvit_edge_l1_supported": (C.c_int, [C.POINTER(LayerDesc)]),
    "kanvit_edge_l1_row_bands": (C.c_int64, [C.POINTER(LayerDesc)]),
    "kanvit_edge_l1_fwd_workspace": (C.c_size_t, [C.POINTER(LayerDesc)]),
    "kanvit_edge_l1_fwd": (C.c_int, [C.POINTER(LayerDesc), _P, _P, _P, _P, _P, C.c_size_t, _P]),
    "kanvit_edge_l1_bwd_workspace": (C.c_size_t, [C.POINTER(LayerDesc)]),
    "kanvit_edge_l1_bwd": (C.c_int, [C.POINTER(LayerDesc), _P, _P, _P, _P, _P, _P, _P, C.c_size_t, _P]),
    "kanvit_bspline_refit_supported": (C.c_int, [C.POINTER(LayerDesc)]),
    "kanvit_bspline_refit_workspace": (C.c_size_t, [C.POINTER(LayerDesc)]),
    "kanvit_bspline_refit_gram": (C.c_int, [C.POINTER(LayerDesc), _P, _P, _P, _P, _P, _P, C.c_size_t, _P]),
    "kanvit_bspline_refit_solve": (C.c_int, [C.POINTER(LayerDesc), _P, _P, _P, _P, _P, _P]),
    "kanvit_bspline_regrid_supported": (C.c_int, [C.POINTER(LayerDesc), C.c_int]),
    "kanvit_bspline_regrid_workspace": (C.c_size_t, [C.POINTER(LayerDesc), C.c_int]),
    "kanvit_bspline_regrid_gram": (C.c_int, [C.POINTER(LayerDesc), C.c_int, _P, _P, _P, _P, _P, _P, C.c_size_t, _P]),
    "kanvit_bspline_regrid_solve": (C.c_int, [C.POINTER(LayerDesc), C.c_int, _P, _P, _P, _P, _P, _P]),
    "kanvit_patch_embed_fwd": (C.c_int, [C.POINTER(LayerDesc), C.POINTER(PatchDesc), _P, _P, _P, _P, _P, _P, _P, _P]),
    "kanvit_patch_embed_fwd_ws": (C.c_int, [C.POINTER(LayerDesc), C.POINTER(PatchDesc), _P, _P, _P, _P, _P, _P, _P, _P, C.c_size_t, _P]),
    "kanvit_patch_embed_bwd_weight_ok": (C.c_int, [C.POINTER(LayerDesc), C.POINTER(PatchDesc)]),
    "kanvit_patch_embed_bwd_weight_workspace": (C.c_size_t, [C.POINTER(LayerDesc), C.POINTER(PatchDesc)]),
    "kanvit_patch_embed_bwd_weight": (C.c_int, [C.POINTER(LayerDesc), C.POINTER(PatchDesc), _P, _P, _P, _P, _P, C.c_size_t, _P]),
    "kanvit_attn_fwd": (C.c_int, [C.POINTER(AttnDesc), _P, _P, _P, _P, _P, _P]),
    "kanvit_attn_bwd_workspace": (C.c_size_t, [C.POINTER(AttnDesc)]),
    "kanvit_attn_bwd": (C.c_int, [C.POINTER(AttnDesc), _P, _P, _P, _P, _P, _P, _P, _P, _P, _P, C.c_size_t, _P]),
    "kanvit_attn_x_fwd": (C.c_int, [C.POINTER(AttnDesc), C.POINTER(AttnExt), _P, _P, _P, _P, _P, _P]),
    "kanvit_attn_x_bwd_workspace": (C.c_size_t, [C.POINTER(AttnDesc), C.POINTER(AttnExt)]),
    "kanvit_attn_x_bwd": (C.c_int, [C.POINTER(AttnDesc), C.POINTER(AttnExt), _P, _P, _P, _P, _P, _P, _P, _P, _P, _P, C.c_size_t, _P]),
    "kanvit_attn_probs": (C.c_int, [C.POINTER(AttnDesc), C.POINTER(AttnExt), _P, _P, _P, C.c_int64, C.c_int64, C.c_int64, C.c_int32, _P]),
    "kanvit_attn_q1_fwd": (C.c_int, [C.POINTER(AttnDesc), C.POINTER(AttnExt), _P, _P, _P, _P, _P, _P]),
    "kanvit_attn_q1_bwd": (C.c_int, [C.POINTER(AttnDesc), C.POINTER(AttnExt), _P, _P, _P, _P, _P, _P, _P, _P, _P, _P]),
    "kanvit_addln_fwd": (C.c_int, [C.c_int64, C.c_int, C.c_float, _P, _P, _P, _P, _P, _P, _P, _P, _P]),
    "kanvit_addln_fwd_ex": (C.c_int, [C.c_int64, C.c_int, C.c_float, _P, _P, C.c_int, _P, _P, _P, _P, C.c_int, _P, _P, _P]),
    "kanvit_addln_bwd_ex": (C.c_int, [C.c_int64, C.c_int, _P, _P, _P, _P, _P, C.c_int, _P, _P, _P, _P, _P, _P, C.c_size_t, _P]),
    "kanvit_addln_bwd_workspace": (C.c_size_t, [C.c_int64, C.c_int]),
    "kanvit_addln_bwd": (C.c_int, [C.c_int64, C.c_int, _P, _P, _P, _P, _P, _P, _P, _P, _P, _P, C.c_size_t, _P]),
    "kanvit_depth_scales": (C.c_int, [C.c_int64, C.c_int, _P, C.c_uint64, _P, _P, _P]),
    "kanvit_addln_sd_fwd": (C.c_int, [C.c_int64, C.c_int, C.c_float, _P, _P, C.c_int, _P, _P, _P, _P, C.c_int, _P, _P, _P, C.c_int64, _P]),
    "kanvit_addln_sd_bwd": (C.c_int, [C.c_int64, C.c_int, _P, _P, _P, _P, _P, C.c_int, _P, _P, _P, C.c_int, _P, _P, _P, C.c_int64, _P, C.c_size_t, _P]),
    "kanvit_relu_bwd_bias_workspace": (C.c_size_t, [C.c_int64, C.c_int]),
    "kanvit_relu_bwd_bias": (C.c_int, [C.c_int64, C.c_int, _P, _P, _P, _P, _P, C.c_size_t, _P]),
    "kanvit_relu_bwd_bias_bf16": (C.c_int, [C.c_int64, C.c_int, _P, _P, _P, _P, _P, C.c_size_t, _P]),
    "kanvit_split3_bf16": (C.c_int, [C.c_int64, C.c_int, _P, _P, C.c_int, _P, C.c_int64, _P, C.c_int, _P]),
    "kanvit_augment_u8_supported": (C.c_int, [C.c_int64, C.c_int, C.c_int, C.c_int, C.c_int, C.c_int]),
    "kanvit_augment_u8": (C.c_int, [_P, _P, _P, _P, _P, _P, _P, C.c_int64, C.c_int64, C.c_int, C.c_int, C.c_int, C.c_int, C.c_int, C.c_int,
                                    C.c_uint64, C.c_uint64, _P]),
    "kanvit_mix_u8": (C.c_int, [_P] * 11 + [C.c_int64, C.c_int64, C.c_int, C.c_int, C.c_int, C.c_int, C.c_int, C.c_int, C.c_uint64, C.c_uint64, _P]),
    "kanvit_resample_u8_supported": (C.c_int, [C.c_int64, C.c_int, C.c_int, C.c_int, C.c_int, C.c_int]),
    "kanvit_resample_u8": (C.c_int, [_P] * 12 + [C.c_int64, C.c_int64, C.c_int, C.c_int, C.c_int, C.c_int, C.c_int, _P]),
    "kanvit_soft_ce": (C.c_int, [_P, C.c_int64, _P, _P, _P, C.c_int64, C.c_int, C.c_float, _P, _P, _P, _P]),
    "kanvit_metrics_update": (C.c_int, [_P, C.c_int, C.c_int64, _P, C.c_int64, C.c_int, C.c_int64, C.c_int64, _P, _P, _P, _P, _P]),
    "kanvit_metrics_auc_pairs_workspace": (C.c_size_t, [C.c_int64, C.c_int]),
    "kanvit_metrics_auc_pairs": (C.c_int, [_P, _P, C.c_int64, C.c_int, C.c_int64, _P, _P, C.c_size_t, _P]),
    "kanvit_optim_max_tensors": (C.c_int, []),
    "kanvit_optim_sumsq_workspace": (C.c_size_t, [C.c_int, _P]),
    "kanvit_optim_sumsq": (C.c_int, [C.c_int, _P, _P, _P, C.c_size_t, _P]),
    "kanvit_optim_begin": (C.c_int, [_P, C.c_int64, C.c_double, _P, _P, _P]),
    "kanvit_optim_adamw": (C.c_int, [C.c_int, _P, _P, _P, _P, _P, _P, _P, _P, C.c_int64, _P, C.c_int64, _P, _P, C.c_int] + [C.c_float] * 7 + [_P]),
}
OPTIM_CHUNK = 4096
DEPTH_MAX_BRANCHES = 64
for _f in FAMILY_NAMES:
    SYMBOLS[f"kanvit_{_f}_fwd"] = (C.c_int, _LAYER_FWD)
    SYMBOLS[f"kanvit_{_f}_bwd_input"] = (C.c_int, _LAYER_BWD_IN)
    SYMBOLS[f"kanvit_{_f}_bwd_weight"] = (C.c_int, _LAYER_BWD_W)
    SYMBOLS[f"kanvit_{_f}_qkv_fwd"] = (C.c_int, _LAYER_FWD)
    SYMBOLS[f"kanvit_{_f}_qkv_bwd_input"] = (C.c_int, _LAYER_BWD_IN)
    SYMBOLS[f"kanvit_{_f}_qkv_bwd_weight"] = (C.c_int, _LAYER_BWD_W)

_lib = None


def lib():
    global _lib
    if _lib is None:
        if not os.path.exists(LIB_PATH):
            raise KanvitError(
                f"{LIB_PATH} not found: build it with `python kan-vit_amd/kanvit/build.py` "
                "(or __graft_entry__.build()). The kanvit ops have no CPU / eager fallback.")
        handle = C.CDLL(LIB_PATH)
        for name, (res, args) in SYMBOLS.items():
            fn = getattr(handle, name)
            fn.restype = res
            fn.argtypes = args
        if handle.kanvit_abi_version() != 7:
            raise KanvitError("libkanvit.so ABI version mismatch")
        _lib = handle
    return _lib


_py_switches = None


def py_switches() -> dict:
    global _py_switches
    if _py_switches is None:
        _py_switches = {"ff": os.environ.get("KANVIT_FF", ""), "no_ff_small": int(bool(os.environ.get("KANVIT_NO_FF_SMALL"))),
                        "no_lnff": int(bool(os.environ.get("KANVIT_NO_LNFF"))),
                        "no_ff_epi": int(bool(os.environ.get("KANVIT_NO_FF_EPILOGUE"))),
                        "no_dfreq_w": int(bool(os.environ.get("KANVIT_NO_DFREQ_W"))),
                        "no_patch_bw": int(bool(os.environ.get("KANVIT_NO_PATCH_BW"))),
                        "no_cls_tail": int(bool(os.environ.get("KANVIT_NO_CLS_TAIL")))}
    return _py_switches


def active_config() -> str:
    ps = py_switches()
    alt = f" lib={LIB_PATH}" if os.environ.get("KANVIT_LIB") else ""
    return lib().kanvit_config().decode() + f" py_ff={ps['ff'] or 'default'} py_no_ff_small={ps['no_ff_small']} py_no_lnff={ps['no_lnff']} py_no_ff_epi={ps['no_ff_epi']} py_no_dfreq_w={ps['no_dfreq_w']} py_no_patch_bw={ps['no_patch_bw']}" + alt + f" py_no_cls_tail={ps['no_cls_tail']}"


def reload_config() -> str:
    global _py_switches
    _py_switches = None
    lib().kanvit_config_reload()
    return active_config()


def check(rc, what):
    if rc != 0:
        msg = lib().kanvit_last_error()
        raise KanvitError(f"{what} failed (code {rc}): {msg.decode() if msg else '?'}")
```

kan-vit_amd/kanvit/ops.py:

```python
from __future__ import annotations

import ctypes as C
from dataclasses import dataclass, replace
from typing import Optional, Tuple

import torch

from . import _lib
from ._lib import BSPLINE, CHEBY, FOURIER, LINEAR, RBF, SINE, AttnDesc, KanvitError, LayerDesc, check


@dataclass(frozen=True)
class LayerCfg:
    family: int
    I: int
    O: int
    G: int
    groups: int = 1
    x_group_mod: int = 1
    spline_order: int = 0
    has_base: int = 0
    rbf_inv_h: float = 0.0
    flags: int = 0
    ln_eps: float = 0.0
    base_act: int = 0

    @property
    def GP(self) -> int:
        return {LINEAR: 1, CHEBY: self.G, BSPLINE: self.G + self.has_base, RBF: self.G + self.has_base,
                SINE: self.G, FOURIER: 2 * self.G}[self.family]

    @property
    def K(self) -> int:
        return self.I * self.GP


class KernelTimer:

    def __init__(self):
        self.records = {}

    def add(self, tag, start, end, flops, nbytes):
        self.records.setdefault(tag, []).append((start, end, flops, nbytes))

    def summary(self):
        torch.cuda.synchronize()
        out = {}
        for tag, recs in self.records.items():
            ms = [s.elapsed_time(e) for s, e, _, _ in recs]
            out[tag] = {"launches": len(recs), "total_ms": sum(ms), "avg_ms": sum(ms) / len(ms),
                        "flops": recs[0][2], "bytes": recs[0][3]}
        return out


timer: Optional[KernelTimer] = None


class _timed:
    def __init__(self, tag, flops=0, nbytes=0):
        self.tag, self.flops, self.nbytes = tag, flops, nbytes

    def __enter__(self):
        if timer is not None:
            self.s = torch.cuda.Event(enable_timing=True)
            self.e = torch.cuda.Event(enable_timing=True)
            self.s.record()
        return self

    def __exit__(self, *exc):
        if timer is not None:
            self.e.record()
            timer.add(self.tag, self.s, self.e, self.flops, self.nbytes)
        return False


def _layer_cost(cfg: "LayerCfg", M: int, kind: str):
    flops = 2 * M * cfg.K * cfg.O * cfg.groups
    xb, yb, wb = M * cfg.x_group_mod * cfg.I, M * cfg.groups * cfg.O, cfg.groups * cfg.K * cfg.O
    nbytes = 4 * {"fwd": xb + yb + wb, "bwd_input": 2 * xb + yb + wb, "bwd_weight": xb + yb + wb}[kind]
    return flops, nbytes


def _ptr(t: Optional[torch.Tensor]):
    return None if t is None else C.c_void_p(t.data_ptr())


def _stream():
    return C.c_void_p(torch.cuda.current_stream().cuda_stream)


def _require_gpu_f32(name: str, t: Optional[torch.Tensor]):
    if t is None:
        return
    if not t.is_cuda:
        raise KanvitError(f"{name} is on {t.device}: the kanvit ops run only on an AMD GPU (no CPU fallback)")
    if t.dtype != torch.float32:
        raise KanvitError(f"{name} has dtype {t.dtype}; the kanvit kernels compute in float32")


SUPPORTED_BASE_ACTIVATIONS = ("nn.SiLU(), F.silu; nn.GELU(), F.gelu; nn.GELU(approximate='tanh'), "
                              "functools.partial(F.gelu, approximate='tanh'); nn.ReLU(), F.relu, torch.relu; "
                              "nn.Tanh(), torch.tanh, F.tanh; nn.Identity()")


def base_activation_code(fn) -> Optional[int]:
    import functools
    import torch.nn.functional as F
    nn = torch.nn
    if isinstance(fn, functools.partial):
        if fn.args or not (fn.func is F.gelu or fn.func is torch._C._nn.gelu):
            return None
        if set(fn.keywords) - {"approximate"}:
            return None
        a = fn.keywords.get("approximate", "none")
        return {"none": _lib.BASE_GELU, "tanh": _lib.BASE_GELU_TANH}.get(a)
    if isinstance(fn, nn.Module):
        t = type(fn)
        if t is nn.SiLU:
            return None if fn.inplace else _lib.BASE_SILU
        if t is nn.GELU:
            return {"none": _lib.BASE_GELU, "tanh": _lib.BASE_GELU_TANH}.get(fn.approximate)
        if t is nn.ReLU:
            return None if fn.inplace else _lib.BASE_RELU
        if t is nn.Tanh:
            return _lib.BASE_TANH
        if t is nn.Identity:
            return _lib.BASE_IDENTITY
        return None
    if fn is F.silu:
        return _lib.BASE_SILU
    if fn is F.gelu or fn is torch._C._nn.gelu:
        return _lib.BASE_GELU
    if fn is F.relu or fn is torch.relu:
        return _lib.BASE_RELU
    if fn is torch.tanh or fn is F.tanh:
        return _lib.BASE_TANH
    return None


def base_act_of(fn) -> int:
    code = base_activation_code(fn)
    if code is None:
        raise NotImplementedError(f"base_activation {fn!r} is not implemented by the fused kernels; supported: "
                                  f"{SUPPORTED_BASE_ACTIVATIONS}")
    return code


def _desc(cfg: LayerCfg, M: int, ldx: int, ldu: int, ldy: int, bp_stride: int) -> LayerDesc:
    return LayerDesc(cfg.family, cfg.groups, cfg.x_group_mod, cfg.I, cfg.O, cfg.G, cfg.spline_order, cfg.has_base,
                     cfg.rbf_inv_h, cfg.flags, M, ldx, ldu, ldy, bp_stride, cfg.ln_eps, cfg.base_act)


def _workspace(nbytes: int, device):
    return torch.empty(max((nbytes + 3) // 4, 4), device=device, dtype=torch.float32)


_NO_SCRATCH = (lambda: 0,)


def _launch(fn, label, device, *args, query=None, null_ws=False, tag=None, cost=(0, 0)):
    with torch.cuda.device(device):
        if query is None:
            tail = (_stream(),)
        else:
            nbytes = int(query[0](*query[1:]))
            ws = None if null_ws and not nbytes else _workspace(nbytes, device)
            tail = (_ptr(ws), C.c_size_t(nbytes), _stream())
        if tag is None or timer is None:
            check(fn(*args, *tail), label)
        else:
            with _timed(tag(nbytes) if callable(tag) else tag, *cost):
                check(fn(*args, *tail), label)


_fwd_f32 = torch.amp.custom_fwd(device_type="cuda", cast_inputs=torch.float32)
_bwd = torch.amp.custom_bwd(device_type="cuda")


def _bf16_tag(tag: str, flags: int) -> str:
    return tag + "_bf16" if flags & _lib.FLAG_BF16_MFMA else tag


def _kan_forward(cfg: LayerCfg, x, u, w, bparams, bias, tag, fused_ln=False):
    for n, t in (("x", x), ("u", u), ("w", w), ("bparams", bparams), ("bias", bias)):
        _require_gpu_f32(n, t)
    x, u, w, bparams, bias = (None if t is None else t.contiguous() for t in (x, u, w, bparams, bias))
    M, ldx = x.shape
    if ldx != cfg.x_group_mod * cfg.I:
        raise KanvitError(f"x has {ldx} columns, expected x_group_mod*I = {cfg.x_group_mod * cfg.I}")
    if tuple(w.shape) != (cfg.groups, cfg.K, cfg.O):
        raise KanvitError(f"packed weight shape {tuple(w.shape)} != {(cfg.groups, cfg.K, cfg.O)}")
    if fused_ln:
        if tuple(bparams.shape) != (cfg.groups, cfg.G + 2 * cfg.I):
            raise KanvitError(f"bparams shape {tuple(bparams.shape)} != {(cfg.groups, cfg.G + 2 * cfg.I)} (centres | gamma | beta)")
        u = torch.empty(M, cfg.x_group_mod, 2, device=x.device, dtype=torch.float32)
    elif u is not None and tuple(u.shape) != (M, cfg.groups * cfg.I):
        raise KanvitError(f"u shape {tuple(u.shape)} != {(M, cfg.groups * cfg.I)}")
    y = torch.empty(M, cfg.groups * cfg.O, device=x.device, dtype=torch.float32)
    d = _desc(cfg, M, ldx, cfg.groups * cfg.I, cfg.groups * cfg.O, 0 if bparams is None else bparams.shape[1])
    L = _lib.lib()
    _launch(L.kanvit_layer_fwd, "kanvit_layer_fwd", x.device, C.byref(d), _ptr(x), _ptr(u), _ptr(w), _ptr(bparams), _ptr(bias), _ptr(y),
            query=(L.kanvit_layer_fwd_workspace, C.byref(d)), null_ws=True,
            tag=_bf16_tag(_tag_prefix(cfg, tag) + "_fwd", cfg.flags), cost=_layer_cost(cfg, M, "fwd"))
    return y, x, u, w, bparams, bias


class _KanLayerFn(torch.autograd.Function):

    @staticmethod
    @_fwd_f32
    def forward(ctx, x, u, w, bparams, bias, cfg: LayerCfg, tag: Optional[str] = None):
        y, x, u, w, bparams, bias = _kan_forward(cfg, x, u, w, bparams, bias, tag)
        ctx.tag = tag
        ctx.cfg = cfg
        ctx.has_u = u is not None
        ctx.has_bp = bparams is not None
        ctx.has_bias = bias is not None
        ctx.save_for_backward(x, u, w, bparams)
        return y

    @staticmethod
    @_bwd
    def backward(ctx, dy):
        x, u, w, bparams = ctx.saved_tensors
        return _kan_backward(ctx.cfg, x, u if ctx.has_u else None, w, bparams, dy.float().contiguous(), ctx.needs_input_grad[:5],
                             ctx.has_u, ctx.has_bias, tag=ctx.tag) + (None, None)


def _tag_prefix(cfg: "LayerCfg", tag: Optional[str]) -> str:
    return tag or ("qkv" if cfg.groups > 1 else "layer")


def _kan_backward(cfg: "LayerCfg", x, u, w, bparams, dy, needs, has_u, has_bias, patch=None, tag=None):
    if patch is not None:
        pd, M = patch
        ldx = cfg.I
        assert not (needs[0] or needs[1]), "the patch form has no input gradient"
    else:
        pd = None
        M, ldx = x.shape
    need_x, need_u, need_w, need_bp, need_b = needs
    stem = _tag_prefix(cfg, tag)
    d = _desc(cfg, M, ldx, cfg.groups * cfg.I, cfg.groups * cfg.O, 0 if bparams is None else bparams.shape[1])
    L = _lib.lib()

    def weight_pass(desc, out, what):
        tag, cost = _bf16_tag(stem + what, cfg.flags), _layer_cost(cfg, M, "bwd_weight")
        if pd is not None:
            _launch(L.kanvit_patch_embed_bwd_weight, "kanvit_patch_embed_bwd_weight", x.device, C.byref(desc), C.byref(pd), _ptr(x),
                    _ptr(bparams), _ptr(dy), _ptr(out), query=(L.kanvit_patch_embed_bwd_weight_workspace, C.byref(desc), C.byref(pd)),
                    tag=tag, cost=cost)
        else:
            _launch(L.kanvit_layer_bwd_weight, "kanvit_layer_bwd_weight", x.device, C.byref(desc), _ptr(x), _ptr(u), _ptr(bparams),
                    _ptr(dy), _ptr(out), query=(L.kanvit_layer_bwd_weight_workspace, C.byref(desc)), tag=tag, cost=cost)

    dx = du = dw = dbp = db = None
    sine_freq = cfg.family == SINE and need_bp
    freq_via_w = False
    if sine_freq and not need_x and (pd is not None or not _lib.py_switches()["no_dfreq_w"]):
        with torch.cuda.device(x.device):
            freq_via_w = bool(L.kanvit_layer_sine_dfreq_ok(C.byref(d)))
    if pd is not None and sine_freq and not freq_via_w:
        raise KanvitError("patch form: SineKAN's frequency gradient needs the register weight-gradient kernel")
    with torch.cuda.device(x.device):
        if need_x or (need_u and has_u) or (sine_freq and not freq_via_w):
            dx = torch.empty_like(x)
            du_buf = torch.empty(M, cfg.groups * cfg.I, device=x.device, dtype=torch.float32) if cfg.family == RBF else None
            dpart = None
            if cfg.family == SINE:
                tiles = int(L.kanvit_layer_dparam_tiles(C.byref(d)))
                dpart = torch.empty(tiles, cfg.groups, cfg.G, device=x.device, dtype=torch.float32)
            _launch(L.kanvit_layer_bwd_input, "kanvit_layer_bwd_input", x.device, C.byref(d), _ptr(x), _ptr(u), _ptr(w), _ptr(bparams),
                    _ptr(dy), _ptr(dx), _ptr(du_buf), _ptr(dpart), query=(L.kanvit_layer_bwd_input_workspace, C.byref(d)), null_ws=True,
                    tag=lambda nb_in: stem + "_bwd_input" + ("_bf16" if nb_in else ""), cost=_layer_cost(cfg, M, "bwd_input"))
            if cfg.family == RBF:
                if has_u:
                    du = du_buf
                else:
                    nshare = cfg.groups // cfg.x_group_mod
                    dx = dx + du_buf.view(M, nshare, cfg.x_group_mod * cfg.I).sum(1)
            if sine_freq:
                dbp = torch.zeros_like(bparams)
                dbp[:, :cfg.G] = dpart.sum(0)
        if need_w:
            dw = torch.empty_like(w)
            weight_pass(d, dw, "_bwd_weight")
        if freq_via_w:
            dq = LayerDesc(*[getattr(d, f) for f, _ in LayerDesc._fields_])
            dq.flags = cfg.flags | _lib.FLAG_SINE_DFREQ
            q = torch.empty_like(w)
            weight_pass(dq, q, "_bwd_freq")
            dbp = torch.zeros_like(bparams)
            dbp[:, :cfg.G] = q.mul_(w).view(cfg.groups, cfg.I, cfg.G, cfg.O).sum((1, 3))
        if need_b and has_bias:
            if pd is not None:
                db = dy[:, pd.prepend_rows:, :].sum((0, 1)).view(1, cfg.O)
            else:
                db = dy.view(M, cfg.groups, cfg.O).sum(0)
    return (dx if need_x else None), (du if need_u else None), dw, dbp, db


def ln_fusable(cfg: "LayerCfg", M: int) -> bool:
    if cfg.family != RBF:
        return False
    d = _desc(_autocast_cfg(cfg), M, cfg.x_group_mod * cfg.I, cfg.groups * cfg.I, cfg.groups * cfg.O,
              cfg.G + 2 * cfg.I)
    return bool(_lib.lib().kanvit_layer_ln_fusable(C.byref(d)))


class _KanLayerLnFn(torch.autograd.Function):

    @staticmethod
    @_fwd_f32
    def forward(ctx, x, w, bparams, bias, cfg: LayerCfg, tag: Optional[str] = None):
        y, x, stats, w, bparams, bias = _kan_forward(cfg, x, None, w, bparams, bias, tag, fused_ln=True)
        ctx.tag = tag
        ctx.cfg = cfg
        ctx.has_bias = bias is not None
        ctx.save_for_backward(x, stats, w, bparams)
        return y

    @staticmethod
    @_bwd
    def backward(ctx, dy):
        x, stats, w, bparams = ctx.saved_tensors
        cfg = ctx.cfg
        need_x, need_w, need_bp, need_b = ctx.needs_input_grad[:4]
        need_ln = need_x or need_bp
        dx, du, dw, _, db = _kan_backward(cfg, x, stats, w, bparams, dy.float().contiguous(),
                                          (need_ln, need_ln, need_w, False, need_b), True, ctx.has_bias, tag=ctx.tag)
        dbp = None
        if need_ln:
            M, I, G = x.shape[0], cfg.I, cfg.G
            d = _desc(cfg, M, x.shape[1], cfg.groups * I, cfg.groups * cfg.O, bparams.shape[1])
            L = _lib.lib()
            dgb = torch.empty(2, cfg.groups, I, device=x.device, dtype=torch.float32)
            _launch(L.kanvit_layer_ln_bwd, "kanvit_layer_ln_bwd", x.device, C.byref(d), _ptr(x), _ptr(stats), _ptr(bparams), _ptr(du),
                    _ptr(dx if need_x else None), _ptr(dgb[0]), _ptr(dgb[1]), query=(L.kanvit_layer_ln_bwd_workspace, C.byref(d)),
                    tag="ln_bwd", cost=(0, 4 * M * (cfg.groups * I + (3 if need_x else 1) * cfg.x_group_mod * I)))
            if need_bp:
                dbp = torch.cat([torch.zeros(cfg.groups, G, device=x.device, dtype=torch.float32), dgb[0], dgb[1]], dim=1)
        return (dx if need_x else None), dw, dbp, db, None, None


def kan_layer_ln(x: torch.Tensor, w: torch.Tensor, cfg: LayerCfg, bparams: torch.Tensor, bias: Optional[torch.Tensor],
                 eps: float, tag: Optional[str] = None) -> torch.Tensor:
    f = cfg.flags | _lib.FLAG_FUSED_LN | _autocast_flags()
    return _KanLayerLnFn.apply(x, w, bparams, bias, replace(cfg, flags=f, ln_eps=float(eps)), tag)


def patchify(images: torch.Tensor, n_patches: int) -> torch.Tensor:
    b, c, h, w = images.shape
    ph, pw = h // n_patches, w // n_patches
    return images.reshape(b, c, n_patches, ph, n_patches, pw).permute(0, 2, 4, 1, 3, 5).reshape(b, n_patches * n_patches, c * ph * pw)


class _PatchEmbedFn(torch.autograd.Function):

    @staticmethod
    @_fwd_f32
    def forward(ctx, images, w, bparams, bias, cls, pos, cfg: LayerCfg, n_patches: int):
        for n, t in (("images", images), ("w", w), ("bparams", bparams), ("bias", bias), ("cls", cls), ("pos", pos)):
            _require_gpu_f32(n, t)
        images = images.contiguous()
        w = w.contiguous()
        B, Cc, H, W = images.shape
        P = n_patches * n_patches
        y = torch.empty(B, P + 1, cfg.O, device=images.device, dtype=torch.float32)
        d = _desc(cfg, B * P, cfg.I, cfg.I, cfg.O, 0 if bparams is None else bparams.shape[1])
        pd = _lib.PatchDesc(Cc, H, W, n_patches, 1, 0)
        bp = None if bparams is None else bparams.contiguous()
        bs = None if bias is None else bias.contiguous()
        cl, po = cls.contiguous(), pos.contiguous()
        L = _lib.lib()
        _launch(L.kanvit_patch_embed_fwd_ws, "kanvit_patch_embed_fwd", images.device, C.byref(d), C.byref(pd), _ptr(images), _ptr(w), _ptr(bp),
                _ptr(bs), _ptr(cl), _ptr(po), _ptr(y), null_ws=True,
                query=(L.kanvit_layer_fwd_workspace, C.byref(d)) if cfg.flags & _lib.FLAG_BF16_MFMA else _NO_SCRATCH,
                tag=_bf16_tag("layer_fwd", cfg.flags), cost=_layer_cost(cfg, B * P, "fwd"))
        ctx.cfg, ctx.n_patches = cfg, n_patches
        ctx.has_bp, ctx.has_bias = bparams is not None, bias is not None
        ctx.save_for_backward(images, w, bp)
        return y

    @staticmethod
    @_bwd
    def backward(ctx, dy):
        images, w, bparams = ctx.saved_tensors
        cfg, P = ctx.cfg, ctx.n_patches ** 2
        dy = dy.float().contiguous()
        B, Cc, H, W = images.shape
        dcls = dy[:, 0, :].sum(0) if ctx.needs_input_grad[4] else None
        needs = (False, False, ctx.needs_input_grad[1], ctx.needs_input_grad[2] and ctx.has_bp, ctx.needs_input_grad[3] and ctx.has_bias)
        pd = _lib.PatchDesc(Cc, H, W, ctx.n_patches, 1, 0)
        d = _desc(cfg, B * P, cfg.I, cfg.I, cfg.O, 0 if bparams is None else bparams.shape[1])
        with torch.cuda.device(images.device):
            gather = bool(_lib.lib().kanvit_patch_embed_bwd_weight_ok(C.byref(d), C.byref(pd))) and not _lib.py_switches()["no_patch_bw"]
        if cfg.family == SINE and _lib.py_switches()["no_dfreq_w"]:
            gather = False
        if gather:
            _, _, dw, dbp, db = _kan_backward(cfg, images, None, w, bparams, dy, needs, False, ctx.has_bias, patch=(pd, B * P))
        else:
            x = patchify(images, ctx.n_patches).reshape(-1, cfg.I)
            dyt = dy[:, 1:, :].reshape(-1, cfg.O)
            _, _, dw, dbp, db = _kan_backward(cfg, x, None, w, bparams, dyt, needs, False, ctx.has_bias)
        return None, dw, dbp, db, dcls, None, None, None


def patch_embed(images, w, cfg: LayerCfg, bparams, bias, cls, pos, n_patches: int) -> torch.Tensor:
    return _PatchEmbedFn.apply(images, w, bparams, bias, cls, pos, _autocast_cfg(cfg), n_patches)


def kan_layer(x: torch.Tensor, w: torch.Tensor, cfg: LayerCfg, u: Optional[torch.Tensor] = None,
              bparams: Optional[torch.Tensor] = None, bias: Optional[torch.Tensor] = None, tag: Optional[str] = None) -> torch.Tensor:
    return _KanLayerFn.apply(x, u, w, bparams, bias, _autocast_cfg(cfg), tag)


EDGE_L1_FAMILIES = (BSPLINE, CHEBY, RBF)


def _edge_l1_desc(cfg: LayerCfg, x: torch.Tensor, bparams) -> LayerDesc:
    M, cols = x.shape
    two = cfg.family == RBF and cfg.has_base
    want = cfg.x_group_mod * cfg.I * (2 if two else 1)
    if cols != want:
        raise KanvitError(f"edge_l1: x has {cols} columns, expected {want}" + (" ([u | x] for RBF with the base column)" if two else ""))
    ldx = max(x.stride(0), cols) if M > 1 else cols
    return _desc(cfg, M, ldx, cfg.x_group_mod * cfg.I if two else 0, cfg.groups * cfg.O, 0 if bparams is None else bparams.shape[1])


class _EdgeL1Fn(torch.autograd.Function):

    @staticmethod
    @_fwd_f32
    def forward(ctx, x, w, bparams, cfg: LayerCfg):
        for n, t in (("x", x), ("w", w), ("bparams", bparams)):
            _require_gpu_f32(n, t)
        if x.dim() != 2:
            raise KanvitError(f"edge_l1: x must be 2-D, got {tuple(x.shape)}")
        if x.stride(1) != 1 or (x.shape[0] > 1 and x.stride(0) < x.shape[1]):
            x = x.contiguous()
        w = w.contiguous()
        bparams = None if bparams is None else bparams.contiguous()
        if tuple(w.shape) != (cfg.groups, cfg.K, cfg.O):
            raise KanvitError(f"packed weight shape {tuple(w.shape)} != {(cfg.groups, cfg.K, cfg.O)}")
        d = _edge_l1_desc(cfg, x, bparams)
        L = _lib.lib()
        A = torch.empty(cfg.groups, cfg.I, cfg.O, device=x.device, dtype=torch.float32)
        _launch(L.kanvit_edge_l1_fwd, "kanvit_edge_l1_fwd", x.device, C.byref(d), _ptr(x), _ptr(w), _ptr(bparams), _ptr(A),
                query=(L.kanvit_edge_l1_fwd_workspace, C.byref(d)), tag="edge_l1_fwd",
                cost=(2 * x.shape[0] * cfg.K * cfg.O * cfg.groups, 4 * (x.numel() + w.numel() + A.numel())))
        ctx.cfg = cfg
        ctx.save_for_backward(x, w, bparams)
        return A

    @staticmethod
    @_bwd
    def backward(ctx, gA):
        x, w, bparams = ctx.saved_tensors
        cfg = ctx.cfg
        gA = gA.float().contiguous()
        d = _edge_l1_desc(cfg, x, bparams)
        L = _lib.lib()
        dw = torch.empty_like(w)
        dx = torch.empty_strided(x.shape, (d.ldx, 1), device=x.device, dtype=torch.float32) if ctx.needs_input_grad[0] else None
        _launch(L.kanvit_edge_l1_bwd, "kanvit_edge_l1_bwd", x.device, C.byref(d), _ptr(x), _ptr(w), _ptr(bparams), _ptr(gA), _ptr(dw), _ptr(dx),
                query=(L.kanvit_edge_l1_bwd_workspace, C.byref(d)), tag="edge_l1_bwd",
                cost=((6 if dx is not None else 4) * x.shape[0] * cfg.K * cfg.O * cfg.groups,
                      4 * ((1 if dx is None else 2) * x.numel() + 2 * w.numel() + gA.numel())))
        return dx, dw, None, None


def edge_l1(x2d: torch.Tensor, w_packed: torch.Tensor, cfg: LayerCfg, bparams: Optional[torch.Tensor] = None) -> torch.Tensor:
    if cfg.family not in EDGE_L1_FAMILIES:
        raise NotImplementedError(f"edge_l1: family {_lib.FAMILY_NAMES[cfg.family]} is not supported (supported: bspline, cheby, rbf)")
    keep = _lib.FLAG_UNIFORM_KNOTS | _lib.FLAG_SHARED_BPARAMS
    if cfg.flags & ~keep:
        cfg = replace(cfg, flags=cfg.flags & keep)
    return _EdgeL1Fn.apply(x2d, w_packed, bparams, cfg)


def l1_entropy_loss(l1: torch.Tensor, regularize_activation: float = 1.0, regularize_entropy: float = 1.0) -> torch.Tensor:
    total = l1.sum((-2, -1), keepdim=True)
    p = l1 / total
    per_layer = regularize_activation * total.squeeze(-1).squeeze(-1) - regularize_entropy * torch.special.xlogy(p, p).sum((-2, -1))
    return per_layer.sum()


def _bspline_fit(who: str, x2d, w_old_packed, cfg: LayerCfg, old_G: int, old_knots, new_knots, keep_old: bool):
    if cfg.family != BSPLINE:
        raise NotImplementedError(f"{who}: family {_lib.FAMILY_NAMES[cfg.family]} has no knot table to refit (bspline only)")
    cfg = replace(cfg, flags=cfg.flags & (_lib.FLAG_UNIFORM_KNOTS | _lib.FLAG_SHARED_BPARAMS))
    for n, t in (("x", x2d), ("w_old", w_old_packed), ("old_knots", old_knots), ("new_knots", new_knots)):
        _require_gpu_f32(n, t)
    x = x2d
    if x.dim() != 2:
        raise KanvitError(f"{who}: x must be 2-D, got {tuple(x.shape)}")
    if x.shape[1] != cfg.x_group_mod * cfg.I:
        raise KanvitError(f"{who}: x has {x.shape[1]} columns, expected {cfg.x_group_mod * cfg.I}")
    if x.stride(1) != 1 or (x.shape[0] > 1 and x.stride(0) < x.shape[1]):
        x = x.contiguous()
    M = x.shape[0]
    ldx = max(x.stride(0), x.shape[1]) if M > 1 else x.shape[1]
    nb, nk = cfg.G, cfg.G + cfg.spline_order + 1
    nbo, nko = old_G, old_G + cfg.spline_order + 1
    w_old = w_old_packed.contiguous()
    if tuple(w_old.shape) != (cfg.groups, cfg.I * nbo, cfg.O):
        raise KanvitError(f"{who}: packed weight shape {tuple(w_old.shape)} != {(cfg.groups, cfg.I * nbo, cfg.O)}" if keep_old else
                          f"{who}: old packed weight shape {tuple(w_old.shape)} != {(cfg.groups, cfg.I * nbo, cfg.O)} (old nb={nbo})")
    old_msg = "{}: old knot table {} does not hold [{}][{}*{}]"
    if not keep_old and (old_knots.dim() < 1 or old_knots.shape[0] != cfg.groups):
        raise KanvitError(old_msg.format(who, tuple(old_knots.shape), cfg.groups, cfg.I, nko))
    old_knots = old_knots.reshape(cfg.groups, -1).contiguous()
    new_knots = new_knots.contiguous()
    bad_old, bad_new = old_knots.shape[1] < cfg.I * nko, tuple(new_knots.shape) != (cfg.x_group_mod, cfg.I, nk)
    if keep_old and (bad_old or bad_new):
        raise KanvitError(f"{who}: knot tables {tuple(old_knots.shape)} / {tuple(new_knots.shape)} do not hold "
                          f"[{cfg.groups}][{cfg.I}*{nk}] / [{cfg.x_group_mod}][{cfg.I}][{nk}]")
    if bad_old:
        raise KanvitError(old_msg.format(who, tuple(old_knots.shape), cfg.groups, cfg.I, nko))
    if bad_new:
        raise KanvitError(f"{who}: new knot table {tuple(new_knots.shape)} != [{cfg.x_group_mod}][{cfg.I}][{nk}]")
    d = _desc(cfg, M, ldx, 0, cfg.groups * cfg.O, old_knots.shape[1])
    L = _lib.lib()
    dev = x.device
    lead = (C.byref(d),) if keep_old else (C.byref(d), C.c_int(old_G))
    gram_n = torch.empty(cfg.x_group_mod, cfg.I, nb, nb, device=dev, dtype=torch.float64)
    gram_c = torch.empty(cfg.groups, cfg.I, nb, nbo, device=dev, dtype=torch.float64)
    w_new = w_old.clone() if keep_old else torch.zeros(cfg.groups, cfg.I * nb, cfg.O, device=dev, dtype=torch.float32)
    ok = torch.empty(cfg.x_group_mod, cfg.I, device=dev, dtype=torch.uint8)
    with torch.cuda.device(dev), _timed(who, 2 * M * cfg.I * nb * (cfg.groups * nbo + cfg.x_group_mod * nb),
                                        4 * (x.numel() + w_old.numel() + w_new.numel())):
        _launch(getattr(L, f"kanvit_{who}_gram"), f"kanvit_{who}_gram", dev, *lead, _ptr(x), _ptr(old_knots), _ptr(new_knots), _ptr(gram_n),
                _ptr(gram_c), query=(getattr(L, f"kanvit_{who}_workspace"), *lead))
        _launch(getattr(L, f"kanvit_{who}_solve"), f"kanvit_{who}_solve", dev, *lead, _ptr(gram_n), _ptr(gram_c), _ptr(w_old), _ptr(w_new),
                _ptr(ok))
    return w_new, ok.bool()


@torch.no_grad()
def bspline_refit(x2d: torch.Tensor, w_old_packed: torch.Tensor, cfg: LayerCfg, old_knots: torch.Tensor,
                  new_knots: torch.Tensor) -> Tuple[torch.Tensor, torch.Tensor]:
    return _bspline_fit("bspline_refit", x2d, w_old_packed, cfg, cfg.G, old_knots, new_knots, keep_old=True)


@torch.no_grad()
def bspline_regrid(x2d: torch.Tensor, w_old_packed: torch.Tensor, cfg_new: LayerCfg, old_G: int, old_knots: torch.Tensor,
                   new_knots: torch.Tensor) -> Tuple[torch.Tensor, torch.Tensor]:
    return _bspline_fit("bspline_regrid", x2d, w_old_packed, cfg_new, int(old_G), old_knots, new_knots, keep_old=False)


_attn_flags = 0


def _attn_build_desc(q, k, v, o, causal: bool, scale: float, flags: int, self_attention: bool) -> AttnDesc:
    B, H, Nq, D = q.shape
    Nk = Nq if self_attention else k.shape[2]
    for n, t, L in (("q", q, Nq), ("k", k, Nk), ("v", v, Nk), ("o", o, Nq)):
        if t.dim() != 4 or tuple(t.shape) != (B, H, L, D):
            if not self_attention:
                raise KanvitError(f"attention: q {tuple(q.shape)}, k {tuple(k.shape)}, v {tuple(v.shape)}, o {tuple(o.shape)} do not agree")
            raise KanvitError(f"attention: {n} has shape {tuple(t.shape)}, expected {(B, H, L, D)} "
                              "(self-attention only: q, k, v and o must agree in batch, heads, length and head size)")
        if t.stride(3) != 1:
            raise KanvitError(f"{n}: innermost dimension must be contiguous")
    return AttnDesc(B, H, Nq, D, int(bool(causal)), float(scale), int(flags), 0,
                    q.stride(0), q.stride(1), q.stride(2), k.stride(0), k.stride(1), k.stride(2),
                    v.stride(0), v.stride(1), v.stride(2), o.stride(0), o.stride(1), o.stride(2))


def _attn_desc(q, k, v, o, causal: bool, scale: float, flags: int = 0) -> AttnDesc:
    return _attn_build_desc(q, k, v, o, causal, scale, flags, True)


def _attn_fits_one_workgroup(N: int, D: int) -> bool:
    if D > 64:
        return False
    ks, npad = (32 if D <= 32 else 64) + 1, (N + 31) // 32 * 32
    return N <= 256 and 4 * (2 * npad * ks + 2 * npad + 4 * 32 * ks) <= 160 * 1024


def _attn_x_flags(flags: int, D: int) -> int:
    return flags & _lib.FLAG_BF16_MFMA if D <= 64 else 0


def _attn_takes_general_kernels(q, k) -> bool:
    return q.dim() == 4 and tuple(k.shape) == tuple(q.shape) and not _attn_fits_one_workgroup(q.shape[2], q.shape[3])


def _attn_fwd(q, k, v, o, causal, scale, flags=0):
    if _attn_takes_general_kernels(q, k):
        return _attn_x_fwd(q, k, v, o, None, causal, scale, flags=_attn_x_flags(flags, q.shape[3]))
    B, H, N, D = q.shape
    lse = torch.empty(B, H, N, device=q.device, dtype=torch.float32)
    d = _attn_desc(q, k, v, o, causal, scale, flags)
    _launch(_lib.lib().kanvit_attn_fwd, "kanvit_attn_fwd", q.device, C.byref(d), _ptr(q), _ptr(k), _ptr(v), _ptr(o), _ptr(lse),
            tag=_bf16_tag("attn_fwd", flags), cost=(4 * B * H * N * N * D, 4 * 4 * B * H * N * D))
    return lse


def _attn_backward(name, descs, q, k, v, o, lse, do, dq, dk, dv, tag, cost):
    if (do.stride() != o.stride()) or dq.stride() != q.stride() or dk.stride() != k.stride() or dv.stride() != v.stride():
        raise KanvitError("attention backward: gradient layouts must match their forward tensors")
    L = _lib.lib()
    lead = tuple(C.byref(t) for t in descs)
    _launch(getattr(L, name), name, q.device, *lead, _ptr(q), _ptr(k), _ptr(v), _ptr(o), _ptr(lse), _ptr(do), _ptr(dq), _ptr(dk), _ptr(dv),
            query=(getattr(L, name + "_workspace"), *lead), tag=tag, cost=cost)


def _attn_bwd(q, k, v, o, lse, do, dq, dk, dv, causal, scale, flags=0):
    if _attn_takes_general_kernels(q, k):
        return _attn_x_bwd(q, k, v, o, lse, do, dq, dk, dv, None, causal, scale, flags=_attn_x_flags(flags, q.shape[3]))
    d = _attn_desc(q, k, v, o, causal, scale, flags)
    B, H, N, D = q.shape
    _attn_backward("kanvit_attn_bwd", (d,), q, k, v, o, lse, do, dq, dk, dv, _bf16_tag("attn_bwd", flags),
                   (10 * B * H * N * N * D, 4 * 9 * B * H * N * D))


def _attn_ext(Nk: int, mask) -> "_lib.AttnExt":
    if mask is None:
        return _lib.AttnExt(Nk, 0, None, 0, 0, 0, 0)
    return _lib.AttnExt(Nk, 0, mask.data_ptr(), mask.stride(0), mask.stride(1), mask.stride(2), mask.stride(3))


def _attn_x_desc(q, k, v, o, mask, causal: bool, scale: float, flags: int = 0):
    for n, t in (("q", q), ("k", k), ("v", v), ("o", o)):
        _require_gpu_f32(n, t)
    d = _attn_build_desc(q, k, v, o, causal, scale, flags, False)
    B, H, Nq, Nk = d.B, d.H, d.N, k.shape[2]
    if mask is not None and (mask.dtype != torch.bool or not mask.is_cuda or tuple(mask.shape) != (B, H, Nq, Nk)):
        raise KanvitError(f"attention mask: need a torch.bool GPU tensor expanded to {(B, H, Nq, Nk)}, got {mask.dtype} {tuple(mask.shape)}")
    return d, _attn_ext(Nk, mask)


def _attn_x_fwd(q, k, v, o, mask, causal, scale, flags=0):
    B, H, Nq, D = q.shape
    lse = torch.empty(B, H, Nq, device=q.device, dtype=torch.float32)
    d, e = _attn_x_desc(q, k, v, o, mask, causal, scale, flags)
    Nk = k.shape[2]
    _launch(_lib.lib().kanvit_attn_x_fwd, "kanvit_attn_x_fwd", q.device, C.byref(d), C.byref(e), _ptr(q), _ptr(k), _ptr(v), _ptr(o), _ptr(lse),
            tag=_bf16_tag("attn_x_fwd", flags), cost=(4 * B * H * Nq * Nk * D, 4 * 2 * B * H * (Nq + Nk) * D))
    return lse


def _attn_x_bwd(q, k, v, o, lse, do, dq, dk, dv, mask, causal, scale, flags=0):
    d, e = _attn_x_desc(q, k, v, o, mask, causal, scale, flags)
    B, H, Nq, D = q.shape
    Nk = k.shape[2]
    _attn_backward("kanvit_attn_x_bwd", (d, e), q, k, v, o, lse, do, dq, dk, dv, _bf16_tag("attn_x_bwd", flags),
                   (14 * B * H * Nq * Nk * D, 4 * 4 * B * H * (Nq + Nk) * D))


class _AttnPackedFn(torch.autograd.Function):

    @staticmethod
    @_fwd_f32
    def forward(ctx, qkv, causal: bool, scale: float, flags: int = 0):
        _require_gpu_f32("qkv", qkv)
        qkv = qkv.contiguous()
        B, N, three, H, D = qkv.shape
        q, k, v = (qkv[:, :, i].permute(0, 2, 1, 3) for i in range(3))
        o = torch.empty(B, N, H, D, device=qkv.device, dtype=torch.float32)
        lse = _attn_fwd(q, k, v, o.permute(0, 2, 1, 3), causal, scale, flags)
        ctx.save_for_backward(qkv, o, lse)
        ctx.causal, ctx.scale, ctx.flags = causal, scale, flags
        return o.view(B, N, H * D)

    @staticmethod
    @_bwd
    def backward(ctx, do):
        do = do.float()
        qkv, o, lse = ctx.saved_tensors
        B, N, _, H, D = qkv.shape
        do = do.contiguous().view(B, N, H, D)
        dqkv = torch.empty_like(qkv)
        q, k, v = (qkv[:, :, i].permute(0, 2, 1, 3) for i in range(3))
        dq, dk, dv = (dqkv[:, :, i].permute(0, 2, 1, 3) for i in range(3))
        _attn_bwd(q, k, v, o.permute(0, 2, 1, 3), lse, do.permute(0, 2, 1, 3), dq, dk, dv, ctx.causal, ctx.scale, ctx.flags)
        return dqkv, None, None, None


class _AttnFn(torch.autograd.Function):

    @staticmethod
    @_fwd_f32
    def forward(ctx, q, k, v, causal: bool, scale: float, flags: int = 0):
        for n, t in (("q", q), ("k", k), ("v", v)):
            _require_gpu_f32(n, t)
        q, k, v = (t if t.stride(3) == 1 else t.contiguous() for t in (q, k, v))
        o = torch.empty(q.shape, device=q.device, dtype=torch.float32)
        lse = _attn_fwd(q, k, v, o, causal, scale, flags)
        ctx.save_for_backward(q, k, v, o, lse)
        ctx.causal, ctx.scale, ctx.flags = causal, scale, flags
        return o

    @staticmethod
    @_bwd
    def backward(ctx, do):
        q, k, v, o, lse = ctx.saved_tensors
        do = do.float().contiguous()
        dq, dk, dv = (torch.empty_strided(t.shape, t.stride(), device=t.device, dtype=t.dtype) for t in (q, k, v))
        _attn_bwd(q, k, v, o, lse, do, dq, dk, dv, ctx.causal, ctx.scale, ctx.flags)
        return dq, dk, dv, None, None, None


def _autocast_flags() -> int:
    on = torch.is_autocast_enabled("cuda") and torch.get_autocast_dtype("cuda") == torch.bfloat16
    return _lib.FLAG_BF16_MFMA if on else 0


def _autocast_cfg(cfg: LayerCfg) -> LayerCfg:
    f = cfg.flags | _autocast_flags()
    return cfg if f == cfg.flags else replace(cfg, flags=f)


def attention_packed(qkv: torch.Tensor, causal: bool = False, scale: Optional[float] = None) -> torch.Tensor:
    return _AttnPackedFn.apply(qkv, causal, qkv.shape[-1] ** -0.5 if scale is None else scale, _autocast_flags())


def attention(q: torch.Tensor, k: torch.Tensor, v: torch.Tensor, causal: bool = False,
              scale: Optional[float] = None) -> torch.Tensor:
    return _AttnFn.apply(q, k, v, causal, q.shape[-1] ** -0.5 if scale is None else scale, _autocast_flags())


class _AttnQ1Fn(torch.autograd.Function):

    @staticmethod
    @_fwd_f32
    def forward(ctx, q0, kv, scale: float):
        _require_gpu_f32("q0", q0)
        _require_gpu_f32("kv", kv)
        if kv.dim() != 5 or kv.shape[2] != 2 or q0.dim() != 3 or (q0.shape[0], q0.shape[1], q0.shape[2]) != (kv.shape[0], kv.shape[3], kv.shape[4]):
            raise KanvitError(f"attention_q1: q0 {tuple(q0.shape)} and kv {tuple(kv.shape)} are not [B, H, D] and [B, N, 2, H, D]")
        q0, kv = q0.contiguous(), kv.contiguous()
        B, N, _, H, D = kv.shape
        o = torch.empty(B, H, D, device=kv.device, dtype=torch.float32)
        p = torch.empty(B, H, N, device=kv.device, dtype=torch.float32)
        d, e = _attn_q1_desc(q0, kv, o, scale)
        _launch(_lib.lib().kanvit_attn_q1_fwd, "kanvit_attn_q1_fwd", kv.device, C.byref(d), C.byref(e), _ptr(q0), _ptr(kv[:, :, 0]),
                _ptr(kv[:, :, 1]), _ptr(o), _ptr(p), tag="attn_q1_fwd", cost=(4 * B * H * N * D, 4 * B * H * (2 * N * D + N + 2 * D)))
        ctx.save_for_backward(q0, kv, o, p)
        ctx.scale = scale
        return o

    @staticmethod
    @_bwd
    def backward(ctx, do):
        q0, kv, o, p = ctx.saved_tensors
        do = do.float().contiguous()
        B, N, _, H, D = kv.shape
        dq = torch.empty_like(q0)
        dkv = torch.empty_like(kv)
        d, e = _attn_q1_desc(q0, kv, o, ctx.scale)
        _launch(_lib.lib().kanvit_attn_q1_bwd, "kanvit_attn_q1_bwd", kv.device, C.byref(d), C.byref(e), _ptr(q0), _ptr(kv[:, :, 0]),
                _ptr(kv[:, :, 1]), _ptr(o), _ptr(p), _ptr(do), _ptr(dq), _ptr(dkv[:, :, 0]), _ptr(dkv[:, :, 1]),
                tag="attn_q1_bwd", cost=(8 * B * H * N * D, 4 * B * H * (4 * N * D + N + 4 * D)))
        return dq, dkv, None


def _attn_q1_desc(q0, kv, o, scale: float):
    B, N, _, H, D = kv.shape
    k = kv[:, :, 0]
    d = AttnDesc(B, H, 1, D, 0, float(scale), 0, 0, q0.stride(0), q0.stride(1), 0, k.stride(0), k.stride(2), k.stride(1),
                 k.stride(0), k.stride(2), k.stride(1), o.stride(0), o.stride(1), 0)
    return d, _attn_ext(N, None)


def attention_q1(q0: torch.Tensor, kv: torch.Tensor, scale: Optional[float] = None) -> torch.Tensor:
    return _AttnQ1Fn.apply(q0, kv, kv.shape[-1] ** -0.5 if scale is None else float(scale))


def expand_attention_mask(mask: Optional[torch.Tensor], q: torch.Tensor, k: torch.Tensor) -> Optional[torch.Tensor]:
    if mask is None:
        return None
    if mask.dim() == 2:
        mask = mask[:, None, None, :]
    return mask.to(device=q.device, dtype=torch.bool).expand(q.shape[0], q.shape[1], q.shape[2], k.shape[2])


def _attn_probs(q, k, mask, causal, scale, rows):
    for n, t in (("q", q), ("k", k)):
        _require_gpu_f32(n, t)
        if t.dim() != 4:
            raise KanvitError(f"attention_probs: {n} has shape {tuple(t.shape)}, expected [B, H, length, D]")
    B, H, Nq, D = q.shape
    if tuple(k.shape[:2]) != (B, H) or k.shape[3] != D:
        raise KanvitError(f"attention_probs: q {tuple(q.shape)} and k {tuple(k.shape)} do not agree in batch, heads and head size")
    Nk = k.shape[2]
    q, k = (t if t.stride(3) == 1 else t.contiguous() for t in (q, k))
    mask = expand_attention_mask(mask, q, k)
    scale = D ** -0.5 if scale is None else scale
    rows = Nq if rows is None else int(rows)
    if not 1 <= rows <= Nq:
        raise KanvitError(f"attention_probs: rows={rows} must be in [1, {Nq}]")
    if B == 0:
        return torch.empty(B, H, rows, Nk, device=q.device, dtype=torch.float32)
    d = AttnDesc(B, H, Nq, D, int(bool(causal)), float(scale), 0, 0, q.stride(0), q.stride(1), q.stride(2),
                 k.stride(0), k.stride(1), k.stride(2), 0, 0, 0, 0, 0, 0)
    e = _attn_ext(Nk, mask)
    p = torch.empty(B, H, rows, Nk, device=q.device, dtype=torch.float32)
    _launch(_lib.lib().kanvit_attn_probs, "kanvit_attn_probs", q.device, C.byref(d), C.byref(e), _ptr(q), _ptr(k), _ptr(p), p.stride(0),
            p.stride(1), p.stride(2), rows, tag="attn_probs", cost=(6 * B * H * rows * Nk * D, 4 * B * H * (rows * Nk + rows * D + Nk * D)))
    return p


@torch.no_grad()
def attention_probs(q: torch.Tensor, k: torch.Tensor, mask: Optional[torch.Tensor] = None, causal: bool = False,
                    scale: Optional[float] = None, rows: Optional[int] = None) -> torch.Tensor:
    with torch.autocast("cuda", enabled=False):
        q, k = (t.float() if t.is_cuda and t.is_floating_point() else t for t in (q, k))
        return _attn_probs(q, k, mask, causal, scale, rows)


@torch.no_grad()
def attention_probs_packed(qkv: torch.Tensor, causal: bool = False, scale: Optional[float] = None,
                           rows: Optional[int] = None) -> torch.Tensor:
    with torch.autocast("cuda", enabled=False):
        if qkv.is_cuda and qkv.is_floating_point():
            qkv = qkv.float()
        _require_gpu_f32("qkv", qkv)
        if qkv.dim() != 5 or qkv.shape[2] != 3:
            raise KanvitError(f"attention_probs_packed: qkv has shape {tuple(qkv.shape)}, expected [B, N, 3, H, D]")
        qkv = qkv.contiguous()
        q, k = (qkv[:, :, i].permute(0, 2, 1, 3) for i in range(2))
        return _attn_probs(q, k, None, causal, scale, rows)


class _AddLayerNormFn(torch.autograd.Function):

    @staticmethod
    @torch.amp.custom_fwd(device_type="cuda")
    def forward(ctx, x, delta, gamma, beta, eps, y_bf16):
        if not x.is_cuda:
            raise KanvitError(f"x is on {x.device}: the kanvit ops run only on an AMD GPU (no CPU fallback)")
        L = _lib.lib()
        D = x.shape[-1]
        x2 = x.float().contiguous().view(-1, D)
        d2 = None
        if delta is not None:
            d2 = (delta if delta.dtype in (torch.float32, torch.bfloat16) else delta.float()).contiguous().view(-1, D)
        M = x2.shape[0]
        y = torch.empty(M, D, device=x.device, dtype=torch.bfloat16 if y_bf16 else torch.float32)
        s = torch.empty_like(x2) if d2 is not None else x2
        mean = torch.empty(M, device=x.device, dtype=torch.float32)
        rstd = torch.empty(M, device=x.device, dtype=torch.float32)
        g, b = gamma.float().contiguous(), beta.float().contiguous()
        _launch(L.kanvit_addln_fwd_ex, "kanvit_addln_fwd", x.device, M, D, float(eps), _ptr(x2), _ptr(d2),
                int(d2 is not None and d2.dtype == torch.bfloat16), _ptr(g), _ptr(b), _ptr(s) if d2 is not None else None, _ptr(y),
                int(bool(y_bf16)), _ptr(mean), _ptr(rstd))
        ctx.save_for_backward(s, g, mean, rstd)
        ctx.delta_dtype = None if d2 is None else d2.dtype
        ctx.shape = x.shape
        return s.view(x.shape), y.view(x.shape)

    @staticmethod
    @torch.amp.custom_bwd(device_type="cuda")
    def backward(ctx, gs, gy):
        s, g, mean, rstd = ctx.saved_tensors
        L = _lib.lib()
        M, D = s.shape
        if gy is None:
            gy2 = torch.zeros_like(s)
        else:
            gy2 = gy.contiguous().view(M, D)
            if gy2.dtype != torch.bfloat16:
                gy2 = gy2.float()
        gs2 = None if gs is None else gs.contiguous().view(M, D).float()
        dx = torch.empty_like(s)
        dxb = torch.empty(M, D, device=s.device, dtype=torch.bfloat16) if ctx.delta_dtype == torch.bfloat16 else None
        dg = torch.empty(D, device=s.device, dtype=torch.float32)
        db = torch.empty(D, device=s.device, dtype=torch.float32)
        _launch(L.kanvit_addln_bwd_ex, "kanvit_addln_bwd", s.device, M, D, _ptr(s), _ptr(g), _ptr(mean), _ptr(rstd), _ptr(gy2),
                int(gy2.dtype == torch.bfloat16), _ptr(gs2), _ptr(dx), _ptr(dxb), _ptr(dg), _ptr(db), query=(L.kanvit_addln_bwd_workspace, M, D))
        dx = dx.view(ctx.shape)
        dd = None if ctx.delta_dtype is None else (dxb.view(ctx.shape) if dxb is not None else dx)
        return dx, dd, dg, db, None, None


class _AddLayerNormScaledFn(torch.autograd.Function):

    @staticmethod
    @torch.amp.custom_fwd(device_type="cuda")
    def forward(ctx, x, delta, row_scale, rows_per_sample, gamma, beta, eps, y_bf16):
        if not x.is_cuda:
            raise KanvitError(f"x is on {x.device}: the kanvit ops run only on an AMD GPU (no CPU fallback)")
        _require_gpu_f32("row_scale", row_scale)
        L = _lib.lib()
        D = x.shape[-1]
        x2 = x.float().contiguous().view(-1, D)
        d2 = (delta if delta.dtype in (torch.float32, torch.bfloat16) else delta.float()).contiguous().view(-1, D)
        M, N = x2.shape[0], int(rows_per_sample)
        sc = row_scale.contiguous().view(-1)
        if d2.shape != x2.shape or N < 1 or M % N or sc.numel() * N != M:
            raise KanvitError(f"add_layernorm(row_scale): x has {M} rows, delta {tuple(delta.shape)}, {sc.numel()} scales x {N} rows per sample")
        y = torch.empty(M, D, device=x.device, dtype=torch.bfloat16 if y_bf16 else torch.float32)
        s = torch.empty_like(x2)
        mean = torch.empty(M, device=x.device, dtype=torch.float32)
        rstd = torch.empty(M, device=x.device, dtype=torch.float32)
        g, b = gamma.float().contiguous(), beta.float().contiguous()
        _launch(L.kanvit_addln_sd_fwd, "kanvit_addln_sd_fwd", x.device, M, D, float(eps), _ptr(x2), _ptr(d2), int(d2.dtype == torch.bfloat16),
                _ptr(g), _ptr(b), _ptr(s), _ptr(y), int(bool(y_bf16)), _ptr(mean), _ptr(rstd), _ptr(sc), N)
        ctx.save_for_backward(s, g, mean, rstd, sc)
        ctx.delta_dtype = d2.dtype
        ctx.n = N
        ctx.shape = x.shape
        return s.view(x.shape), y.view(x.shape)

    @staticmethod
    @torch.amp.custom_bwd(device_type="cuda")
    def backward(ctx, gs, gy):
        s, g, mean, rstd, sc = ctx.saved_tensors
        L = _lib.lib()
        M, D = s.shape
        if gy is None:
            gy2 = torch.zeros_like(s)
        else:
            gy2 = gy.contiguous().view(M, D)
            if gy2.dtype != torch.bfloat16:
                gy2 = gy2.float()
        gs2 = None if gs is None else gs.contiguous().view(M, D).float()
        dx = torch.empty_like(s)
        dd = torch.empty(M, D, device=s.device, dtype=ctx.delta_dtype)
        dg = torch.empty(D, device=s.device, dtype=torch.float32)
        db = torch.empty(D, device=s.device, dtype=torch.float32)
        _launch(L.kanvit_addln_sd_bwd, "kanvit_addln_sd_bwd", s.device, M, D, _ptr(s), _ptr(g), _ptr(mean), _ptr(rstd), _ptr(gy2),
                int(gy2.dtype == torch.bfloat16), _ptr(gs2), _ptr(dx), _ptr(dd), int(dd.dtype == torch.bfloat16), _ptr(dg), _ptr(db),
                _ptr(sc), ctx.n, query=(L.kanvit_addln_bwd_workspace, M, D))
        return dx.view(ctx.shape), dd.view(ctx.shape), None, None, dg, db, None, None


def add_layernorm(x: torch.Tensor, delta: Optional[torch.Tensor], norm: torch.nn.LayerNorm, y_bf16: bool = False,
                  row_scale: Optional[torch.Tensor] = None, rows_per_sample: Optional[int] = None):
    D = x.shape[-1]
    if row_scale is not None:
        if delta is None:
            raise ValueError("add_layernorm: row_scale scales delta, and delta is None")
        if x.dim() == 3 and rows_per_sample in (None, x.shape[1]):
            rows_per_sample = x.shape[1]
        elif x.dim() != 2 or rows_per_sample is None:
            raise ValueError(f"add_layernorm(row_scale): x is [B, N, d], or 2-D with rows_per_sample; got {tuple(x.shape)}, rows_per_sample={rows_per_sample}")
    if norm.weight is None or norm.bias is None or len(norm.normalized_shape) != 1 or D % 4 or D > 1024 or D < 4:
        if row_scale is not None:
            delta = (row_scale.repeat_interleave(int(rows_per_sample)).view(*x.shape[:-1], 1) * delta).to(delta.dtype)
        s = x if delta is None else x + delta
        return s, norm(s)
    if row_scale is not None:
        return _AddLayerNormScaledFn.apply(x, delta, row_scale, int(rows_per_sample), norm.weight, norm.bias, norm.eps, bool(y_bf16))
    return _AddLayerNormFn.apply(x, delta, norm.weight, norm.bias, norm.eps, bool(y_bf16))


def depth_scales(B: int, keep, seed: int, counter: torch.Tensor, out: Optional[torch.Tensor] = None) -> torch.Tensor:
    keep = [float(k) for k in keep]
    n = len(keep)
    if not torch.is_tensor(counter) or not counter.is_cuda or counter.dtype != torch.int64 or counter.numel() != 1:
        raise KanvitError("depth_scales: counter is a one-element int64 tensor on the GPU")
    B = int(B)
    if out is None:
        out = torch.empty(n, max(B, 0), device=counter.device, dtype=torch.float32)
    elif not out.is_cuda or out.dtype != torch.float32 or tuple(out.shape) != (n, B) or not out.is_contiguous():
        raise KanvitError(f"depth_scales: out is a contiguous float32 [{n}, {B}] tensor on the GPU")
    host = (C.c_float * max(n, 1))(*keep)
    _launch(_lib.lib().kanvit_depth_scales, "kanvit_depth_scales", counter.device, B, n, C.cast(host, C.c_void_p),
            C.c_uint64(int(seed) & 0xFFFFFFFFFFFFFFFF), _ptr(counter), _ptr(out))
    return out


def depth_keep(B: int, keep, seed: int, counter: int) -> torch.Tensor:
    import numpy as np
    from .data import _mix
    m64 = 0xFFFFFFFFFFFFFFFF
    base = _mix((_mix(int(seed) & m64) + int(counter)) & m64)
    out = np.zeros((len(keep), int(B)), dtype=np.float32)
    for j, k in enumerate(keep):
        k32 = np.float32(k)
        if not 0.0 < float(k32) <= 1.0:
            raise ValueError(f"depth_keep: keep[{j}]={k} is outside (0, 1]")
        thr = int(np.rint(np.float64(k32) * 16777216.0))
        inv = np.float32(1.0) / k32
        for b in range(int(B)):
            if (_mix((base + (j << 32) + b) & m64) >> 40) < thr:
                out[j, b] = inv
    return torch.from_numpy(out)


def augment_u8(images: torch.Tensor, labels: Optional[torch.Tensor], idx: torch.Tensor, lut: torch.Tensor, pad=0, flip: bool = False,
               seed: int = 0, epoch: int = 0, return_params: bool = False, out: Optional[torch.Tensor] = None):
    for name, t, dt in (("images", images, torch.uint8), ("labels", labels, torch.int64), ("idx", idx, torch.int64), ("lut", lut, torch.float32),
                        ("out", out, torch.float32)):
        if t is None:
            continue
        if not t.is_cuda:
            raise KanvitError(f"augment_u8: {name} is on {t.device}: the kanvit ops run only on an AMD GPU (no CPU fallback)")
        if t.device != images.device:
            raise KanvitError(f"augment_u8: {name} is on {t.device}, images on {images.device}")
        if t.dtype != dt:
            raise KanvitError(f"augment_u8: {name} has dtype {t.dtype}, expected {dt}")
        if not t.is_contiguous():
            raise KanvitError(f"augment_u8: {name} is not contiguous")
    if images.dim() not in (3, 4):
        raise KanvitError(f"augment_u8: images has shape {tuple(images.shape)}, expected [N, H, W, C] or [N, H, W]")
    N, H, W = (int(v) for v in images.shape[:3])
    Cn = int(images.shape[3]) if images.dim() == 4 else 1
    pad_y, pad_x = (int(pad), int(pad)) if isinstance(pad, int) else (int(pad[0]), int(pad[1]))
    if idx.dim() != 1:
        raise KanvitError(f"augment_u8: idx has shape {tuple(idx.shape)}, expected [B]")
# ... 313 lines not shown
```

Measured before the change: 1628.

## Save attention probabilities in forward and reuse them in backward

The N=197 (13-tile) f32 attention forward now writes the normalized softmax probabilities to a per-head 208x208 buffer. The backward kernel reads them back instead of reloading K and Q and recomputing QK^T and the exponentials. This trades the recompute MFMAs for extra global memory traffic and storage, about 170KB per head. An environment variable turns it off.

Result: no change. 1634 (median of 6 runs) (+0.4%).

```diff
diff --git a/include/kanvit.h b/include/kanvit.h
--- a/include/kanvit.h
+++ b/include/kanvit.h
@@ -146,6 +146,14 @@
 int kanvit_attn_bwd(const kanvit_attn_desc* d, const float* q, const float* k, const float* v,
                     const float* o, const float* lse, const float* d_o,
                     float* dq, float* dk, float* dv, void* workspace, size_t workspace_bytes, void* stream);
+
+size_t kanvit_attn_sp_bytes(const kanvit_attn_desc* d);
+int kanvit_attn_fwd_sp(const kanvit_attn_desc* d, const float* q, const float* k, const float* v,
+                       float* o, float* lse, float* p, size_t p_bytes, void* stream);
+int kanvit_attn_bwd_sp(const kanvit_attn_desc* d, const float* q, const float* k, const float* v,
+                       const float* o, const float* lse, const float* d_o,
+                       float* dq, float* dk, float* dv, const float* p, size_t p_bytes,
+                       void* workspace, size_t workspace_bytes, void* stream);
 
 #define KANVIT_ATTN_X_MAX_D 128
 typedef struct kanvit_attn_ext {
diff --git a/kan-vit_amd/csrc/attention.hip b/kan-vit_amd/csrc/attention.hip
--- a/kan-vit_amd/csrc/attention.hip
+++ b/kan-vit_amd/csrc/attention.hip
@@ -2299,16 +2299,43 @@
 }
 #endif
 
+size_t kanvit_attn_sp_bytes(const kanvit_attn_desc* d) {
+    if (!d || d->B < 0 || d->H < 1 || d->N < 1 || d->D < 1 || d->N > KANVIT_ATTN_MAX_N) return 0;
+    const AttnFwdPlan f = plan_attn_fwd(d, 0);
+    const AttnBwdPlan b = plan_attn_bwd(d, AttnAlign{});
+    if (f.form != ATTN_FWD_16 || f.nkt != KV_ATTN16_TILES || b.form != ATTN_BWD_16) return 0;
+    return sizeof(float) * (size_t)d->B * d->H * KV_ATTN16_NP * KV_ATTN16_NP;
+}
+
+static int check_sp(const kanvit_attn_desc* d, const void* p, size_t p_bytes, const char* who) {
+    if (!p) return 0;
+    if ((uintptr_t)p % 16) return kv_fail(KANVIT_EINVAL, "%s: the probability buffer must be 16-byte aligned", who);
+    const size_t need = kanvit_attn_sp_bytes(d);
+    if (p_bytes < need) return kv_fail(KANVIT_ENOMEM, "%s: probability buffer %zu bytes < required %zu", who, p_bytes, need);
+    return 0;
+}
+
 int kanvit_attn_fwd(const kanvit_attn_desc* d, const float* q, const float* k, const float* v, float* o, float* lse,
                     void* stream) {
+    return kanvit_attn_fwd_sp(d, q, k, v, o, lse, nullptr, 0, stream);
+}
+
+int kanvit_attn_fwd_sp(const kanvit_attn_desc* d, const float* q, const float* k, const float* v, float* o, float* lse,
+                       float* p_save, size_t p_bytes, void* stream) {
     if (int rc = check_desc(d, "kanvit_attn_fwd")) return rc;
     if (!q || !k || !v || !o) return kv_fail(KANVIT_EINVAL, "kanvit_attn_fwd: null q/k/v/o");
+    if (int rc = check_sp(d, p_save, p_bytes, "kanvit_attn_fwd_sp")) return rc;
     if (d->B == 0) return 0;
     AttnArgs a = make_args(d);
     a.q = q; a.k = k; a.v = v; a.out = o; a.lse = lse;
     a.vec = a.vec && (((uintptr_t)q | (uintptr_t)k | (uintptr_t)v) % 16 == 0);
     hipStream_t st = (hipStream_t)stream;
     const AttnFwdPlan p = plan_attn_fwd(d, (uintptr_t)q | (uintptr_t)k | (uintptr_t)v | (uintptr_t)o);
+    if (p_save && kanvit_attn_sp_bytes(d)) {
+        if (p.form != ATTN_FWD_16 || p.nkt != KV_ATTN16_TILES)
+            return kv_fail(KANVIT_EINVAL, "kanvit_attn_fwd_sp: q, k, v and o must be 16-byte aligned to save the probabilities");
+        a.p_out = p_save;
+    }
     switch (p.form) {
         case ATTN_FWD_SMALL:
             hipLaunchKernelGGL(attn_small_fwd_kernel, dim3(p.grid), dim3(256), 0, st, a);
@@ -2330,9 +2357,16 @@
 int kanvit_attn_bwd(const kanvit_attn_desc* d, const float* q, const float* k, const float* v, const float* o,
                     const float* lse, const float* d_o, float* dq, float* dk, float* dv, void* workspace,
                     size_t workspace_bytes, void* stream) {
+    return kanvit_attn_bwd_sp(d, q, k, v, o, lse, d_o, dq, dk, dv, nullptr, 0, workspace, workspace_bytes, stream);
+}
+
+int kanvit_attn_bwd_sp(const kanvit_attn_desc* d, const float* q, const float* k, const float* v, const float* o,
+                       const float* lse, const float* d_o, float* dq, float* dk, float* dv, const float* p_saved, size_t p_bytes,
+                       void* workspace, size_t workspace_bytes, void* stream) {
     if (int rc = check_desc(d, "kanvit_attn_bwd")) return rc;
     if (!q || !k || !v || !o || !lse || !d_o || !dq || !dk || !dv)
         return kv_fail(KANVIT_EINVAL, "kanvit_attn_bwd: null argument");
+    if (int rc = check_sp(d, p_saved, p_bytes, "kanvit_attn_bwd_sp")) return rc;
     if (d->B == 0) return 0;
     const uintptr_t in = (uintptr_t)q | (uintptr_t)k | (uintptr_t)v | (uintptr_t)d_o;
     const AttnBwdPlan p = plan_attn_bwd(d, AttnAlign{in | (uintptr_t)dq | (uintptr_t)dk | (uintptr_t)dv, (uintptr_t)o, (uintptr_t)lse});
@@ -2344,6 +2378,7 @@
     a.ds = p.ds != ATTN_DS_NONE ? (float*)((char*)workspace + (sizeof(float) * (size_t)d->B * d->H * d->N + 15) / 16 * 16) : nullptr;
     a.vec = a.vec && in % 16 == 0;
     a.third = !p.delta;
+    a.p_in = (p.form == ATTN_BWD_16 && kanvit_attn_sp_bytes(d)) ? p_saved : nullptr;
     hipStream_t st = (hipStream_t)stream;
     switch (p.form) {
         case ATTN_BWD_SMALL:
diff --git a/kan-vit_amd/csrc/attention16.hip b/kan-vit_amd/csrc/attention16.hip
--- a/kan-vit_amd/csrc/attention16.hip
+++ b/kan-vit_amd/csrc/attention16.hip
@@ -395,6 +395,14 @@
             asm volatile("s_waitcnt lgkmcnt(0)" ::: "memory");
             a16_signal(cnt_s, lane);
         }
+        float* pp_main = nullptr;
+        if constexpr (NKT == A16_MAXT && !BF && !CAUSAL) {
+            if (a.p_out && has_tile) {
+                int l = lane;
+                asm volatile("" : "+v"(l));
+                pp_main = a.p_out + (size_t)bh * (KV_ATTN16_NP * KV_ATTN16_NP) + (16 * wave + (l & 15)) * KV_ATTN16_NP + 4 * (l >> 4);
+            }
+        }
         if (has_tile) {
 #pragma unroll
             for (int dt = 0; dt < 4; ++dt) oacc[dt] = f32x4{0.0f, 0.0f, 0.0f, 0.0f};
@@ -430,6 +438,10 @@
 #pragma unroll
                     for (int dt = 0; dt < 4; ++dt) oacc[dt] = a16_mfma(fv[t % 3][dt], sacc[j][r], oacc[dt]);
                     __builtin_amdgcn_sched_barrier(0);
+                    if constexpr (NKT == A16_MAXT && !CAUSAL && r == 3) {
+                        if (pp_main)
+                            *reinterpret_cast<f32x4*>(pp_main + 16 * j) = f32x4{sacc[j][0] * inv, sacc[j][1] * inv, sacc[j][2] * inv, sacc[j][3] * inv};
+                    }
                 });
             }
             o_bh = bh;
@@ -451,6 +463,16 @@
             if (cl < N) {
                 *reinterpret_cast<f32x4*>(a.out + bi * a.osb + hi * a.osh + cl * (int)a.osn + 16 * (l >> 4) + 4 * wave) = t * cinv;
                 if (wave == 0 && l < 16 && a.lse) a.lse[(long long)bh * N + cl] = mx * a.scale + logf(sum);
+            }
+            if constexpr (NKT == A16_MAXT && !BF && !CAUSAL) {
+                if (a.p_out) {
+                    const float cz = cl < N ? cinv : 0.0f;
+                    float* pp = a.p_out + (size_t)bh * (KV_ATTN16_NP * KV_ATTN16_NP) + cl * KV_ATTN16_NP + 16 * kb0 + 4 * (l >> 4);
+#pragma unroll
+                    for (int jj = 0; jj < 4; ++jj)
+                        if (jj < kb1 - kb0)
+                            *reinterpret_cast<f32x4*>(pp + 16 * jj) = f32x4{cacc[jj][0] * cz, cacc[jj][1] * cz, cacc[jj][2] * cz, cacc[jj][3] * cz};
+                }
             }
         }
         ++item;
@@ -506,7 +528,7 @@
 }
 __device__ __forceinline__ void b16_signal(unsigned* c, int lane, unsigned n = 1u) { a16_signal(c, lane, n); }
 
-template <int NTL, bool BF>
+template <int NTL, bool BF, bool SP>
 __device__ __forceinline__ void attn16_bwd_body(const AttnArgs& a, float* __restrict__ smem, const int lane, const int wave) {
     constexpr int D = A16_D;
     constexpr bool UNITS = (NTL == 1);
@@ -520,6 +542,7 @@
     const int T = B16_NT * nh;
     const int kt0 = UNITS ? 10 + (wave - 5) : 2 * wave;
     const int u = wave - 5;
+    static_assert(!(SP && BF), "the bf16 mode recomputes");
 
     auto head_of = [&](int k) { return (int)blockIdx.x + k * (int)gridDim.x; };
     auto slot6 = [&](int X) { return X % B16_NSL; };
@@ -583,12 +606,13 @@
             const float* vp = a.v + bi * a.vsb + hi * a.vsh + key * (int)a.vsn + 16 * (l >> 4);
 #pragma unroll
             for (int i = 0; i < 4; ++i) {
-                const f32x4 k4 = *reinterpret_cast<const f32x4*>(kp + 4 * i);
                 const f32x4 v4 = *reinterpret_cast<const f32x4*>(vp + 4 * i);
 #pragma unroll
-                for (int e = 0; e < 4; ++e) {
-                    kf[t][4 * i + e] = k4[e];
-                    vf[t][4 * i + e] = v4[e];
+                for (int e = 0; e < 4; ++e) vf[t][4 * i + e] = v4[e];
+                if constexpr (!SP) {
+                    const f32x4 k4 = *reinterpret_cast<const f32x4*>(kp + 4 * i);
+#pragma unroll
+                    for (int e = 0; e < 4; ++e) kf[t][4 * i + e] = k4[e];
                 }
             }
             if constexpr (BF) {
@@ -599,6 +623,23 @@
                 }
             }
         }
+    };
+    float pn[NTL][4];
+    auto load_p = [&](int kk, int ss) {
+        int l = lane;
+        asm volatile("" : "+v"(l));
+        const float* pp = a.p_in + (size_t)head_of(kk) * (KV_ATTN16_NP * KV_ATTN16_NP) + (16 * ss) * KV_ATTN16_NP + 16 * kt0
+                          + ((l >> 4) * (4 * KV_ATTN16_NP) + (l & 15));
+#pragma unroll
+        for (int t = 0; t < NTL; ++t)
+#pragma unroll
+            for (int r = 0; r < 4; ++r) pn[t][r] = pp[r * KV_ATTN16_NP + 16 * t];
+    };
+    auto settle_p = [&]() {
+#pragma unroll
+        for (int t = 0; t < NTL; ++t)
+#pragma unroll
+            for (int r = 0; r < 4; ++r) asm volatile("" : "+v"(pn[t][r]));
     };
     auto unit_tile = [&](int it) -> int { return it < 4 ? u + 3 * it : (u == 1 ? B16_NT - 1 : B16_NT); };
     float ku[UNITS ? 5 : 1][16];
@@ -665,8 +706,10 @@
         load_ku(0);
     }
     load_kv(0);
+    if constexpr (SP) load_p(0, 0);
     zero_acc();
     asm volatile("s_waitcnt vmcnt(0)" ::: "memory");
+    if constexpr (SP) settle_p();
     __syncthreads();
     if (wave == 0) form_delta(0);
     if (threadIdx.x == 0) {
@@ -711,6 +754,7 @@
         B16_CLK_PHASE(7)
         if constexpr (UNITS) {
             asm volatile("s_waitcnt vmcnt(0)" ::: "memory");
+            if constexpr (SP) settle_p();
             B16_CLK_PHASE(11)
             if (u == 0 && G >= B16_LAG + 1) reduce_dq(G - B16_LAG - 1);
             if (G >= B16_LAG) {
@@ -768,6 +812,17 @@
             }
         }
         if (G >= T) continue;
+        float pc[NTL][4];
+        if constexpr (SP) {
+#pragma unroll
+            for (int t = 0; t < NTL; ++t)
+#pragma unroll
+                for (int r = 0; r < 4; ++r) pc[t][r] = pn[t][r];
+            if (G + 1 < T) {
+                if (s + 1 == B16_NT) load_p(k + 1, 0);
+                else load_p(k, s + 1);
+            }
+        }
         if constexpr (!UNITS) {
             if (G + 1 < T && wave == (G + 1) % 5) {
                 b16_wait(cnt + BC_READY + slot6(G + 1), 5u * (unsigned)((G + 1) / B16_NSL + 1));
@@ -792,10 +847,11 @@
             f32x4 fq[4], fd[4], fo[4], fq2[4];
 #pragma unroll
             for (int i = 0; i < 4; ++i) {
-                fq[i] = *reinterpret_cast<const f32x4*>(sl + ko[i]);
+                if constexpr (!SP) fq[i] = *reinterpret_cast<const f32x4*>(sl + ko[i]);
                 fd[i] = *reinterpret_cast<const f32x4*>(sl + 1024 + ko[i]);
             }
-            const f32x4 ls4 = *reinterpret_cast<const f32x4*>(sl + 3072 + 4 * gg);
+            f32x4 ls4;
+            if constexpr (!SP) ls4 = *reinterpret_cast<const f32x4*>(sl + 3072 + 4 * gg);
 #pragma unroll
             for (int r = 0; r < 4; ++r) {
                 fo[r] = *reinterpret_cast<const f32x4*>(sl + 1024 + vo[r]);
@@ -819,6 +875,13 @@
                         sP[t] = a16_mfma_bf(ad, vfb[t][c], sP[t]);
                     }
                 }
+            } else if constexpr (SP) {
+#pragma unroll
+                for (int i = 0; i < 4; ++i)
+#pragma unroll
+                    for (int e = 0; e < 4; ++e)
+#pragma unroll
+                        for (int t = 0; t < NTL; ++t) sP[t] = a16_mfma(fd[i][e], vf[t][4 * i + e], sP[t]);
             } else
 #pragma unroll
             for (int i = 0; i < 4; ++i)
@@ -840,6 +903,15 @@
             b16_wait(cnt + BC_DELTA + slot, (unsigned)(G / B16_NSL + 1));
             const f32x4 dl4 = *reinterpret_cast<const f32x4*>(sl + 3072 + 64 + 4 * gg);
             float pr[NTL][4], ds[NTL][4];
+            if constexpr (SP) {
+#pragma unroll
+                for (int t = 0; t < NTL; ++t)
+#pragma unroll
+                    for (int r = 0; r < 4; ++r) {
+                        pr[t][r] = pc[t][r];
+                        ds[t][r] = pc[t][r] * (sP[t][r] - dl4[r]) * a.scale;
+                    }
+            } else
 #pragma unroll
             for (int t = 0; t < NTL; ++t)
 #pragma unroll
@@ -905,6 +977,7 @@
                 asm volatile("s_waitcnt vmcnt(0)" ::: "memory");
                 b16_signal(cnt + BC_READY + slot6(XL), lane);
             }
+            if constexpr (SP) settle_p();
             B16_CLK_PHASE(11)
             if (XI < T && !(B16_ABLATE & 16)) {
                 if (XI >= B16_NSL) b16_wait(cnt + BC_DONE + slot6(XI), (unsigned)B16_NW * (unsigned)(XI / B16_NSL));
@@ -927,8 +1000,15 @@
     const int tid = threadIdx.x, lane = tid & 63, wave = __builtin_amdgcn_readfirstlane(tid >> 6);
     for (int e = tid * 4; e < b16_lds_floats(); e += B16_THREADS * 4) *reinterpret_cast<f32x4*>(smem + e) = f32x4{0.0f, 0.0f, 0.0f, 0.0f};
     __syncthreads();
-    if (wave < 5) attn16_bwd_body<2, BF>(a, smem, lane, wave);
-    else attn16_bwd_body<1, BF>(a, smem, lane, wave);
+    if constexpr (!BF) {
+        if (a.p_in) {
+            if (wave < 5) attn16_bwd_body<2, false, true>(a, smem, lane, wave);
+            else attn16_bwd_body<1, false, true>(a, smem, lane, wave);
+            return;
+        }
+    }
+    if (wave < 5) attn16_bwd_body<2, BF, false>(a, smem, lane, wave);
+    else attn16_bwd_body<1, BF, false>(a, smem, lane, wave);
 }
 
 static_assert(B16_NT == KV_ATTN16_TILES && A16_MAXT == KV_ATTN16_TILES && sizeof(float) * b16_lds_floats() <= 160 * 1024, "the backward's tiles and LDS");
diff --git a/kan-vit_amd/csrc/attention_common.h b/kan-vit_amd/csrc/attention_common.h
--- a/kan-vit_amd/csrc/attention_common.h
+++ b/kan-vit_amd/csrc/attention_common.h
@@ -16,6 +16,8 @@
     float* dv;
     float* delta;
     float* ds;
+    float* p_out;
+    const float* p_in;
     long long qsb, qsh, qsn, ksb, ksh, ksn, vsb, vsh, vsn, osb, osh, osn;
     int B, H, N, D, causal, nkt, vec;
     int third;
@@ -60,6 +62,7 @@
 
 constexpr int KV_ATTN16_TILES = 13;
 int kv_attn16_tiles(const kanvit_attn_desc* d);
+constexpr int KV_ATTN16_NP = 16 * KV_ATTN16_TILES;
 size_t kv_attn16_fwd_lds(int N);
 size_t kv_attn16_bwd_lds();
 int kv_attn16_launch_fwd(const AttnArgs& a, const AttnFwdPlan& p, hipStream_t st);
diff --git a/kan-vit_amd/kanvit/_lib.py b/kan-vit_amd/kanvit/_lib.py
--- a/kan-vit_amd/kanvit/_lib.py
+++ b/kan-vit_amd/kanvit/_lib.py
@@ -98,7 +98,10 @@
     "kanvit_attn_fwd": (C.c_int, [C.POINTER(AttnDesc), _P, _P, _P, _P, _P, _P]),
     "kanvit_attn_bwd_workspace": (C.c_size_t, [C.POINTER(AttnDesc)]),
     "kanvit_attn_bwd": (C.c_int, [C.POINTER(AttnDesc), _P, _P, _P, _P, _P, _P, _P, _P, _P, _P, C.c_size_t, _P]),
-    "kanvit_attn_x_fwd": (C.c_int, [C.POINTER(AttnDesc), C.POINTER(AttnExt), _P, _P, _P, _P, _P, _P]),
+    "kanvit_attn_sp_bytes": (C.c_size_t, [C.POINTER(AttnDesc)]),
+    "kanvit_attn_fwd_sp": (C.c_int, [C.POINTER(AttnDesc), _P, _P, _P, _P, _P, _P, C.c_size_t, _P]),
+    "kanvit_attn_bwd_sp": (C.c_int, [C.POINTER(AttnDesc), _P, _P, _P, _P, _P, _P, _P, _P, _P, _P, C.c_size_t, _P, C.c_size_t, _P]),
+    "kanvit_attn_x_fwd": (C.c_int,[C.POINTER(AttnDesc), C.POINTER(AttnExt), _P, _P, _P, _P, _P, _P]),
     "kanvit_attn_x_bwd_workspace": (C.c_size_t, [C.POINTER(AttnDesc), C.POINTER(AttnExt)]),
     "kanvit_attn_x_bwd": (C.c_int, [C.POINTER(AttnDesc), C.POINTER(AttnExt), _P, _P, _P, _P, _P, _P, _P, _P, _P, _P, C.c_size_t, _P]),
     "kanvit_attn_probs": (C.c_int, [C.POINTER(AttnDesc), C.POINTER(AttnExt), _P, _P, _P, C.c_int64, C.c_int64, C.c_int64, C.c_int32, _P]),
diff --git a/kan-vit_amd/kanvit/ops.py b/kan-vit_amd/kanvit/ops.py
--- a/kan-vit_amd/kanvit/ops.py
+++ b/kan-vit_amd/kanvit/ops.py
@@ -1,6 +1,7 @@
 from __future__ import annotations
 
 import ctypes as C
+import os
 from dataclasses import dataclass, replace
 from typing import Optional, Tuple
 
@@ -587,33 +588,46 @@
     return q.dim() == 4 and tuple(k.shape) == tuple(q.shape) and not _attn_fits_one_workgroup(q.shape[2], q.shape[3])
 
 
-def _attn_fwd(q, k, v, o, causal, scale, flags=0):
+save_attn_probs = not os.environ.get("KANVIT_NO_ATTN_SP")
+
+
+def _attn_fwd(q, k, v, o, causal, scale, flags=0, save_p=None):
     if _attn_takes_general_kernels(q, k):
-        return _attn_x_fwd(q, k, v, o, None, causal, scale, flags=_attn_x_flags(flags, q.shape[3]))
+        lse = _attn_x_fwd(q, k, v, o, None, causal, scale, flags=_attn_x_flags(flags, q.shape[3]))
+        return lse if save_p is None else (lse, None)
     B, H, N, D = q.shape
     lse = torch.empty(B, H, N, device=q.device, dtype=torch.float32)
     d = _attn_desc(q, k, v, o, causal, scale, flags)
-    _launch(_lib.lib().kanvit_attn_fwd, "kanvit_attn_fwd", q.device, C.byref(d), _ptr(q), _ptr(k), _ptr(v), _ptr(o), _ptr(lse),
+    L = _lib.lib()
+    p, nbytes = None, 0
+    if save_p and save_attn_probs and not any(t.data_ptr() % 16 for t in (q, k, v, o)):
+        nbytes = int(L.kanvit_attn_sp_bytes(C.byref(d)))
+        if nbytes:
+            p = torch.empty(nbytes // (4 * 208 * 208), 208, 208, device=q.device, dtype=torch.float32)
+    fn, extra = ("kanvit_attn_fwd", ()) if p is None else ("kanvit_attn_fwd_sp", (_ptr(p), C.c_size_t(nbytes)))
+    _launch(getattr(L, fn), fn, q.device, C.byref(d), _ptr(q), _ptr(k), _ptr(v), _ptr(o), _ptr(lse), *extra,
             tag=_bf16_tag("attn_fwd", flags), cost=(4 * B * H * N * N * D, 4 * 4 * B * H * N * D))
-    return lse
-
-
-def _attn_backward(name, descs, q, k, v, o, lse, do, dq, dk, dv, tag, cost):
+    return lse if save_p is None else (lse, p)
+
+
+def _attn_backward(name, descs, q, k, v, o, lse, do, dq, dk, dv, tag, cost, p=None):
     if (do.stride() != o.stride()) or dq.stride() != q.stride() or dk.stride() != k.stride() or dv.stride() != v.stride():
         raise KanvitError("attention backward: gradient layouts must match their forward tensors")
     L = _lib.lib()
     lead = tuple(C.byref(t) for t in descs)
-    _launch(getattr(L, name), name, q.device, *lead, _ptr(q), _ptr(k), _ptr(v), _ptr(o), _ptr(lse), _ptr(do), _ptr(dq), _ptr(dk), _ptr(dv),
-            query=(getattr(L, name + "_workspace"), *lead), tag=tag, cost=cost)
-
-
-def _attn_bwd(q, k, v, o, lse, do, dq, dk, dv, causal, scale, flags=0):
+    extra = () if p is None else (_ptr(p), C.c_size_t(p.numel() * 4))
+    fn = name if p is None else name + "_sp"
+    _launch(getattr(L, fn), fn, q.device, *lead, _ptr(q), _ptr(k), _ptr(v), _ptr(o), _ptr(lse), _ptr(do), _ptr(dq), _ptr(dk), _ptr(dv),
+            *extra, query=(getattr(L, name + "_workspace"), *lead), tag=tag, cost=cost)
+
+
+def _attn_bwd(q, k, v, o, lse, do, dq, dk, dv, causal, scale, flags=0, p=None):
     if _attn_takes_general_kernels(q, k):
         return _attn_x_bwd(q, k, v, o, lse, do, dq, dk, dv, None, causal, scale, flags=_attn_x_flags(flags, q.shape[3]))
     d = _attn_desc(q, k, v, o, causal, scale, flags)
     B, H, N, D = q.shape
     _attn_backward("kanvit_attn_bwd", (d,), q, k, v, o, lse, do, dq, dk, dv, _bf16_tag("attn_bwd", flags),
-                   (10 * B * H * N * N * D, 4 * 9 * B * H * N * D))
+                   (10 * B * H * N * N * D, 4 * 9 * B * H * N * D), p=p)
 
 
 def _attn_ext(Nk: int, mask) -> "_lib.AttnExt":
@@ -660,8 +674,8 @@
         B, N, three, H, D = qkv.shape
         q, k, v = (qkv[:, :, i].permute(0, 2, 1, 3) for i in range(3))
         o = torch.empty(B, N, H, D, device=qkv.device, dtype=torch.float32)
-        lse = _attn_fwd(q, k, v, o.permute(0, 2, 1, 3), causal, scale, flags)
-        ctx.save_for_backward(qkv, o, lse)
+        lse, p = _attn_fwd(q, k, v, o.permute(0, 2, 1, 3), causal, scale, flags, save_p=ctx.needs_input_grad[0])
+        ctx.save_for_backward(qkv, o, lse, *(() if p is None else (p,)))
         ctx.causal, ctx.scale, ctx.flags = causal, scale, flags
         return o.view(B, N, H * D)
 
@@ -669,13 +683,14 @@
     @_bwd
     def backward(ctx, do):
         do = do.float()
-        qkv, o, lse = ctx.saved_tensors
+        qkv, o, lse, *p = ctx.saved_tensors
         B, N, _, H, D = qkv.shape
         do = do.contiguous().view(B, N, H, D)
         dqkv = torch.empty_like(qkv)
         q, k, v = (qkv[:, :, i].permute(0, 2, 1, 3) for i in range(3))
         dq, dk, dv = (dqkv[:, :, i].permute(0, 2, 1, 3) for i in range(3))
-        _attn_bwd(q, k, v, o.permute(0, 2, 1, 3), lse, do.permute(0, 2, 1, 3), dq, dk, dv, ctx.causal, ctx.scale, ctx.flags)
+        _attn_bwd(q, k, v, o.permute(0, 2, 1, 3), lse, do.permute(0, 2, 1, 3), dq, dk, dv, ctx.causal, ctx.scale, ctx.flags,
+                  p=p[0] if p else None)
         return dqkv, None, None, None
 
 
@@ -688,18 +703,18 @@
             _require_gpu_f32(n, t)
         q, k, v = (t if t.stride(3) == 1 else t.contiguous() for t in (q, k, v))
         o = torch.empty(q.shape, device=q.device, dtype=torch.float32)
-        lse = _attn_fwd(q, k, v, o, causal, scale, flags)
-        ctx.save_for_backward(q, k, v, o, lse)
+        lse, p = _attn_fwd(q, k, v, o, causal, scale, flags, save_p=any(ctx.needs_input_grad[:3]))
+        ctx.save_for_backward(q, k, v, o, lse, *(() if p is None else (p,)))
         ctx.causal, ctx.scale, ctx.flags = causal, scale, flags
         return o
 
     @staticmethod
     @_bwd
     def backward(ctx, do):
-        q, k, v, o, lse = ctx.saved_tensors
+        q, k, v, o, lse, *p = ctx.saved_tensors
         do = do.float().contiguous()
         dq, dk, dv = (torch.empty_strided(t.shape, t.stride(), device=t.device, dtype=t.dtype) for t in (q, k, v))
-        _attn_bwd(q, k, v, o, lse, do, dq, dk, dv, ctx.causal, ctx.scale, ctx.flags)
+        _attn_bwd(q, k, v, o, lse, do, dq, dk, dv, ctx.causal, ctx.scale, ctx.flags, p=p[0] if p else None)
         return dq, dk, dv, None, None, None
 
 
```
